# PeterSutor/ADMM-Project

Hardware: AMD Instinct MI355X
Metric: ADMM iterations/sec (lasso 100k x 10k, fp64) (higher is better)
Workload: dtype f64; 1 GPU; lasso.m cached-factor loop, D 100000x10000 fp64, rho=1, lassotest.m recipe seed=1, domaxiters=1, objevals=0, xsolve=inverse; rows=100000, cols=10000, parallelism=rows1

## Files before the change

admm-project_amd/_lib.py:

```python
from __future__ import annotations

import ctypes as C
import os

_HERE = os.path.dirname(os.path.abspath(__file__))
LIB_PATH = os.path.join(_HERE, "libadmm_hip.so")

ABI_VERSION = 5

OK, E_INVALID, E_UNSUPPORTED, E_DEVICE, E_NUMERIC, E_COMM, E_CAPACITY = 0, -1, -2, -3, -4, -5, -6

PROB_LASSO, PROB_LASSO_CONSENSUS, PROB_LAD, PROB_HUBERFIT = 1, 2, 3, 4
PROB_LINEARSVM, PROB_TOTALVARIATION, PROB_QP_BOUNDED, PROB_BASISPURSUIT = 5, 6, 7, 8
PROB_MODEL, PROB_LINEARPROGRAM, PROB_QP_STANDARD, PROB_TV2D = 9, 10, 11, 12
PROB_COVSEL = 13
LOSS_HINGE, LOSS_01, LOSS_HINGE_OBJ01, LOSS_LOGISTIC = 0, 1, 2, 3
LOSS_SQHINGE = 5


def loss_code(text):
    if text in ("hinge", "01"):
        return LOSS_HINGE if text == "hinge" else LOSS_01
    if isinstance(text, str) and text.lower() == "logistic":
        return LOSS_LOGISTIC
# ... 254 lines not shown
 SLM_F_DERR) = range(1, 9)


class LassoMultiDesc(C.Structure):
    _fields_ = [("struct_size", C.c_int32), ("K", C.c_int32), ("m", C.c_int64), ("n", C.c_int64), ("D", _dp),
                ("ldD", C.c_int64), ("S", _dp), ("ns", C.c_int32), ("device", C.c_int32), ("rho", C.c_double),
                ("xsolve", C.c_int32), ("reserved0", C.c_int32), ("lam", _dp), ("ridge", _dp),
                ("nonneg", C.POINTER(C.c_int32)), ("weights", _dp), ("comm", C.c_void_p)]


class LassoMultiOptions(C.Structure):
    _fields_ = [("struct_size", C.c_int32), ("maxiters", C.c_int32), ("rho", C.c_double), ("abstol", C.c_double),
                ("reltol", C.c_double), ("relax", C.c_double), ("fast", C.c_int32), ("convtest", C.c_int32),
                ("domaxiters", C.c_int32), ("objevals", C.c_int32), ("check_every", C.c_int32),
                ("nodualerror", C.c_int32), ("x0", _dp), ("z0", _dp), ("u0", _dp)]


class LassoMultiSummary(C.Structure):
    _fields_ = [("steps", C.c_int32), ("stopped_early", C.c_int32), ("objopt", C.c_double), ("xsolve", C.c_int32),
                ("reserved0", C.c_int32)]


(LM_F_XOPT, LM_F_ZOPT, LM_F_UOPT, LM_F_PNORM, LM_F_PERR, LM_F_OBJEVALS, LM_F_DNORM, LM_F_DERR) = range(1, 9)


class CovselMultiDesc(C.Structure):
    _fields_ = [("struct_size", C.c_int32), ("K", C.c_int32), ("m", C.c_int64), ("n", C.c_int64), ("D", _dp),
                ("ldD", C.c_int64), ("S", _dp), ("lam", _dp), ("device", C.c_int32), ("reserved0", C.c_int32),
                ("comm", C.c_void_p)]


class CovselMultiOptions(C.Structure):
    _fields_ = [("struct_size", C.c_int32), ("maxiters", C.c_int32), ("rho", C.c_double), ("abstol", C.c_double),
                ("reltol", C.c_double), ("relax", C.c_double), ("fast", C.c_int32), ("convtest", C.c_int32),
                ("domaxiters", C.c_int32), ("objevals", C.c_int32), ("check_every", C.c_int32),
                ("nodualerror", C.c_int32), ("rhos", _dp), ("z0", _dp), ("u0", _dp)]


class CovselMultiSummary(C.Structure):
    _fields_ = [("steps", C.c_int32), ("stopped_early", C.c_int32), ("objopt", C.c_double),
                ("jacobi_sweeps", C.c_int32), ("reserved0", C.c_int32)]


(CM_F_XOPT, CM_F_ZOPT, CM_F_UOPT, CM_F_PNORM, CM_F_PERR, CM_F_OBJEVALS, CM_F_DNORM, CM_F_DERR, CM_F_COV) = range(1, 10)
COVSEL_SMALL_MAX = 96


class L1ClassDesc(C.Structure):
    _fields_ = [("struct_size", C.c_int32), ("K", C.c_int32), ("m", C.c_int64), ("n", C.c_int64), ("D", _dp),
                ("ldD", C.c_int64), ("ELL", _dp), ("nell", C.c_int32), ("device", C.c_int32), ("C", C.c_double),
                ("xsolve", C.c_int32), ("reserved0", C.c_int32), ("loss", C.POINTER(C.c_int32)), ("lam", _dp),
                ("ridge", _dp), ("nonneg", C.POINTER(C.c_int32)), ("l1weights", _dp), ("comm", C.c_void_p)]


class L1ClassOptions(C.Structure):
    _fields_ = list(LassoMultiOptions._fields_)


class L1ClassSummary(C.Structure):
    _fields_ = list(LassoMultiSummary._fields_)


(L1C_F_XOPT, L1C_F_ZOPT, L1C_F_UOPT, L1C_F_PNORM, L1C_F_PERR, L1C_F_OBJEVALS, L1C_F_DNORM, L1C_F_DERR) = range(1, 9)


class SparseL1ClassDesc(C.Structure):
    _fields_ = [("struct_size", C.c_int32), ("K", C.c_int32), ("D", C.POINTER(SparseDesc)), ("ELL", _dp),
                ("nell", C.c_int32), ("device", C.c_int32), ("C", C.c_double), ("xsolve", C.c_int32),
                ("reserved0", C.c_int32), ("loss", C.POINTER(C.c_int32)), ("lam", _dp), ("ridge", _dp),
                ("nonneg", C.POINTER(C.c_int32)), ("l1weights", _dp), ("comm", C.c_void_p)]


class SparseL1ClassOptions(C.Structure):
    _fields_ = list(SparseRegOptions._fields_)


class SparseL1ClassSummary(C.Structure):
    _fields_ = [("steps", C.c_int32), ("stopped_early", C.c_int32), ("objopt", C.c_double), ("xsolve", C.c_int32),
                ("reserved0", C.c_int32), ("cg_iters_total", C.c_int64), ("cg_capped_updates", C.c_int64)]


FIELD_NUMERIC, FIELD_TEXT, FIELD_HANDLE, FIELD_SPARSE, FIELD_OTHER = 0, 1, 2, 3, 4
RES_FETCH, RES_SCALAR, RES_START = 0, 1, 2
STORAGE_FP64, STORAGE_COMPACT = 0, 1
F_WVALS = 23
F_COVSEL_S = 24
F_TV2D_ROW_STAGE = 25
F_SPARSE_NNZ = 26
TV2D_ROWS_AUTO, TV2D_ROWS_GREEN, TV2D_ROWS_COOP, TV2D_ROWS_DCT, TV2D_ROWS_THOMAS = range(5)
TV2D_ROWS_NAMES = ("cg", "green", "coop", "dct", "thomas")


class AdmmError(RuntimeError):
    def __init__(self, code, message):
        super().__init__(f"[admm_hip {code}] {message}")
        self.code = code


_SIGNATURES = {
    "admm_abi_version": (C.c_int, []),
    "admm_last_error": (C.c_char_p, []),
    "admm_device_count": (C.c_int, [C.POINTER(C.c_int)]),
    "admm_device_info": (C.c_int, [C.c_int, C.c_char_p, C.c_size_t, C.POINTER(C.c_int64), C.POINTER(C.c_int32)]),
    "admm_options_default": (None, [C.POINTER(Options)]),
    "admm_problem_desc_default": (None, [C.POINTER(ProblemDesc)]),
    "admm_engine_create": (C.c_int, [C.POINTER(ProblemDesc), C.POINTER(C.c_void_p)]),
    "admm_engine_create_sparse": (C.c_int, [C.POINTER(ProblemDesc), C.POINTER(SparseDesc), C.POINTER(C.c_void_p)]),
    "admm_engine_set_callbacks": (C.c_int, [C.c_void_p, PROX_CALLBACK, C.c_void_p, PROX_CALLBACK, C.c_void_p,
                                            OBJ_CALLBACK, C.c_void_p]),
    "admm_engine_set_operators": (C.c_int, [C.c_void_p, OPERATOR_CALLBACK, C.c_void_p, OPERATOR_CALLBACK, C.c_void_p]),
    "admm_engine_set_constraint_b": (C.c_int, [C.c_void_p, C.POINTER(C.c_double), C.c_int64, C.c_int64, C.c_int32,
                                               C.c_double, OPERATOR_CALLBACK, C.c_void_p]),
    "admm_engine_set_groups": (C.c_int, [C.c_void_p, C.POINTER(C.c_int64), C.c_int32, _dp]),
    "admm_engine_set_penalty": (C.c_int, [C.c_void_p, C.POINTER(PenaltyDesc)]),
    "admm_engine_get_penalty": (C.c_int, [C.c_void_p, C.POINTER(PenaltyDesc), C.POINTER(C.c_int32)]),
    "admm_engine_set_loss": (C.c_int, [C.c_void_p, C.POINTER(LossDesc)]),
    "admm_engine_get_loss": (C.c_int, [C.c_void_p, C.POINTER(LossDesc), C.POINTER(C.c_int32)]),
    "admm_engine_set_svm_cost": (C.c_int, [C.c_void_p, C.POINTER(SvmCostDesc)]),
    "admm_engine_get_svm_cost": (C.c_int, [C.c_void_p, C.POINTER(SvmCostDesc), C.POINTER(C.c_int32)]),
    "admm_engine_set_tv2d_isotropic": (C.c_int, [C.c_void_p, C.c_int32]),
    "admm_engine_run": (C.c_int, [C.c_void_p, C.POINTER(Options), C.POINTER(RunSummary)]),
    "admm_engine_fetch": (C.c_int, [C.c_void_p, C.c_int, _dp, C.c_size_t, C.POINTER(C.c_size_t)]),
    "admm_engine_set_hooks": (C.c_int, [C.c_void_p, ALTU_CALLBACK, C.c_void_p, NORMS_CALLBACK, C.c_void_p]),
    "admm_engine_info": (C.c_int, [C.c_void_p, C.POINTER(EngineInfo)]),
    "admm_engine_xsolve_storage": (C.c_int, [C.c_void_p, C.POINTER(C.c_int32), C.POINTER(C.c_int64),
                                             C.POINTER(C.c_double), C.POINTER(C.c_double), C.POINTER(C.c_double)]),
    "admm_xsolve_compact_accept": (C.c_int, [C.c_double, C.c_double, C.c_double]),
    "admm_tv2d_row_stage": (C.c_int, [C.c_int64, C.c_int64, C.c_double]),
    "admm_tv2d_rows_green_taps": (C.c_int, [C.c_double]),
    "admm_dct_tables": (C.c_int, [C.c_int64, _dp, _dp, _dp, _dp, _dp, C.POINTER(C.c_int64)]),
    "admm_engine_setup_seconds": (C.c_int, [C.c_void_p, C.POINTER(C.c_double)]),
    "admm_engine_kernel_time": (C.c_int, [C.c_void_p, C.c_int, C.POINTER(C.c_double), C.POINTER(C.c_int64)]),
    "admm_engine_set_profiling": (C.c_int, [C.c_void_p, C.c_int]),
    "admm_engine_set_profiling_stride": (C.c_int, [C.c_void_p, C.c_int]),
    "admm_engine_destroy": (None, [C.c_void_p]),
    "admm_binding_create": (C.c_int, [C.c_char_p, C.POINTER(Field), C.c_int32, C.POINTER(Field), C.c_int32,
                                      C.POINTER(C.c_void_p)]),
    "admm_binding_destroy": (None, [C.c_void_p]),
    "admm_binding_desc": (C.POINTER(ProblemDesc), [C.c_void_p]),
    "admm_binding_sparse": (C.POINTER(SparseDesc), [C.c_void_p]),
    "admm_binding_get_info": (C.c_int, [C.c_void_p, C.POINTER(BindingInfo)]),
    "admm_binding_apply": (C.c_int, [C.c_void_p, C.c_void_p]),
    "admm_binding_options": (C.c_int, [C.c_void_p, C.POINTER(Field), C.c_int32, C.POINTER(Field), C.c_int32,
                                       C.POINTER(Options)]),
    "admm_binding_results": (C.c_int, [C.c_void_p, C.POINTER(Options), C.POINTER(RunSummary), C.POINTER(ResultField),
                                       C.c_int32, C.POINTER(C.c_int32)]),
    "admm_memcpy_d2h": (C.c_int, [C.c_void_p, C.c_void_p, C.c_size_t, C.c_void_p]),
    "admm_memcpy_h2d": (C.c_int, [C.c_void_p, C.c_void_p, C.c_size_t, C.c_void_p]),
    "admm_op_gemv_n": (C.c_int, [_dp, C.c_int64, C.c_int64, C.c_int64, _dp, _dp]),
    "admm_op_gemv_t": (C.c_int, [_dp, C.c_int64, C.c_int64, C.c_int64, _dp, C.c_int64, C.c_int32, _dp, C.c_int64]),
    "admm_op_spmv": (C.c_int, [C.POINTER(SparseDesc), C.c_int, _dp, _dp]),
    "admm_op_gram": (C.c_int, [_dp, C.c_int64, C.c_int64, C.c_int64, C.c_double, _dp]),
    "admm_op_cholesky": (C.c_int, [_dp, C.c_int64, C.c_int64]),
    "admm_op_trsv_pair": (C.c_int, [_dp, C.c_int64, C.c_int64, _dp, _dp]),
    "admm_op_soft_threshold": (C.c_int, [_dp, C.c_int64, C.c_double, _dp]),
    "admm_op_pair_soft_threshold": (C.c_int, [_dp, C.c_int64, C.c_double, _dp]),
    "admm_op_group_soft_threshold": (C.c_int, [_dp, C.c_int64, C.POINTER(C.c_int64), C.c_int32, _dp, C.c_double, _dp]),
    "admm_op_penalty_prox": (C.c_int, [_dp, C.c_int64, C.POINTER(C.c_int64), C.c_int32, _dp, C.c_double,
                                       C.POINTER(PenaltyDesc), C.c_double, _dp]),
    "admm_op_loss_prox": (C.c_int, [_dp, C.c_int64, C.c_int32, C.POINTER(LossDesc), C.c_double, _dp]),
    "admm_op_svm_prox": (C.c_int, [_dp, _dp, C.c_int64, C.c_int32, C.c_double, C.c_double, C.POINTER(SvmCostDesc), _dp]),
    "admm_op_symv": (C.c_int, [_dp, C.c_int64, C.c_int64, _dp, C.c_int32, C.c_int64, C.c_int32, _dp]),
    "admm_op_symv_compact": (C.c_int, [_dp, C.c_int64, C.c_int64, _dp, C.c_int32, C.c_int64, C.c_int32, _dp, _dp,
                                       C.c_int64]),
    "admm_op_symv_batch": (C.c_int, [_dp, C.c_int64, C.c_int64, C.c_int32, _dp, C.c_int64, C.c_int64, _dp, C.c_int64]),
    "admm_op_gemm": (C.c_int, [C.c_int32, C.c_int32, C.c_int64, C.c_int64, C.c_int64, C.c_double, _dp, C.c_int64, _dp,
                               C.c_int64, C.c_double, _dp, C.c_int64, C.c_int32]),
    "admm_op_trtri": (C.c_int, [_dp, C.c_int64, C.c_int64, _dp, C.c_int64]),
    "admm_op_llt_apply": (C.c_int, [_dp, C.c_int64, C.c_int64, _dp, _dp]),
    "admm_op_dct_cols": (C.c_int, [_dp, C.c_int64, C.c_int64, C.c_int32, _dp]),
    "admm_op_tv2d_rows": (C.c_int, [_dp, C.c_int64, C.c_int64, C.c_double, C.c_int32, _dp]),
    "admm_op_tv2d_xsolve": (C.c_int, [_dp, C.c_int64, C.c_int64, C.c_double, C.c_int32, _dp]),
    "admm_op_consensus_tail": (C.c_int, [C.c_int32, C.c_int64, C.c_int32, C.c_int32, C.c_double, C.c_double, _dp, _dp,
                                         _dp, _dp, _dp, _dp, _dp, C.c_int32, _dp, _dp, _dp, _dp, _dp, _dp]),
    "admm_comm_unique_id": (C.c_int, [C.c_char_p]),
    "admm_comm_init": (C.c_int, [C.c_char_p, C.c_int, C.c_int, C.c_int, C.c_int, C.POINTER(C.c_void_p)]),
    "admm_comm_info": (C.c_int, [C.c_void_p, C.POINTER(C.c_int), C.POINTER(C.c_int), C.POINTER(C.c_int)]),
    "admm_comm_allreduce_sum": (C.c_int, [C.c_void_p, _dp, C.c_size_t]),
    "admm_comm_measure_latency": (C.c_int, [C.c_void_p, C.c_size_t, C.c_int, C.POINTER(C.c_double)]),
    "admm_comm_destroy": (None, [C.c_void_p]),
    "admm_comm_init_all": (C.c_int, [C.c_int, C.POINTER(C.c_int), C.c_int, C.POINTER(C.c_void_p)]),
    "admm_engine_create_all": (C.c_int, [C.c_int, C.POINTER(ProblemDesc), C.POINTER(C.c_void_p)]),
    "admm_engine_run_all": (C.c_int, [C.c_int, C.POINTER(C.c_void_p), C.POINTER(Options), C.c_int,
                                      C.POINTER(RunSummary)]),
    "admm_svm_ovr_desc_default": (None, [C.POINTER(SvmOvrDesc)]),
    "admm_svm_ovr_options_default": (None, [C.POINTER(SvmOvrOptions)]),
    "admm_svm_ovr_create": (C.c_int, [C.POINTER(SvmOvrDesc), C.POINTER(C.c_void_p)]),
    "admm_svm_ovr_run": (C.c_int, [C.c_void_p, C.POINTER(SvmOvrOptions), C.POINTER(SvmOvrSummary),
                                   C.POINTER(C.c_double)]),
    "admm_svm_ovr_fetch": (C.c_int, [C.c_void_p, C.c_int, _dp, C.c_size_t, C.POINTER(C.c_size_t)]),
    "admm_svm_ovr_set_cost": (C.c_int, [C.c_void_p, _dp, _dp]),
    "admm_svm_ovr_chunk": (C.c_int, []),
    "admm_svm_ovr_destroy": (None, [C.c_void_p]),
    "admm_reg_multi_desc_default": (None, [C.POINTER(RegMultiDesc)]),
    "admm_reg_multi_options_default": (None, [C.POINTER(RegMultiOptions)]),
    "admm_reg_multi_create": (C.c_int, [C.POINTER(RegMultiDesc), C.POINTER(C.c_void_p)]),
    "admm_reg_multi_run": (C.c_int, [C.c_void_p, C.POINTER(RegMultiOptions), C.POINTER(RegMultiSummary),
                                     C.POINTER(C.c_double)]),
    "admm_reg_multi_fetch": (C.c_int, [C.c_void_p, C.c_int, _dp, C.c_size_t, C.POINTER(C.c_size_t)]),
    "admm_reg_multi_set_weights": (C.c_int, [C.c_void_p, _dp]),
    "admm_reg_multi_launches": (C.c_int, [C.c_void_p, C.POINTER(C.c_int64)]),
    "admm_reg_multi_chunk": (C.c_int, []),
    "admm_reg_multi_destroy": (None, [C.c_void_p]),
    "admm_op_spmm": (C.c_int, [C.POINTER(SparseDesc), C.c_int, C.c_int, _dp, _dp]),
    "admm_op_spmm_weighted": (C.c_int, [C.POINTER(SparseDesc), C.c_int32, _dp, _dp, C.c_int32, C.POINTER(C.c_int32),
                                        C.POINTER(C.c_int32), _dp]),
    "admm_op_spmm_cg": (C.c_int, [C.POINTER(SparseDesc), C.c_int32, _dp, _dp, C.c_double, C.c_double, C.c_int32,
                                  C.c_int32, C.POINTER(C.c_int32), _dp, _dp, C.POINTER(C.c_int64),
                                  C.POINTER(C.c_int32)]),
    "admm_sparse_svm_desc_default": (None, [C.POINTER(SparseSvmDesc)]),
    "admm_sparse_svm_options_default": (None, [C.POINTER(SparseSvmOptions)]),
    "admm_sparse_svm_create": (C.c_int, [C.POINTER(SparseSvmDesc), C.POINTER(C.c_void_p)]),
    "admm_sparse_svm_run": (C.c_int, [C.c_void_p, C.POINTER(SparseSvmOptions), C.POINTER(SparseSvmSummary),
                                      C.POINTER(C.c_double)]),
    "admm_sparse_svm_fetch": (C.c_int, [C.c_void_p, C.c_int, _dp, C.c_size_t, C.POINTER(C.c_size_t)]),
    "admm_sparse_svm_set_cost": (C.c_int, [C.c_void_p, _dp, _dp]),
    "admm_sparse_svm_chunk": (C.c_int, []),
    "admm_sparse_svm_destroy": (None, [C.c_void_p]),
    "admm_sparse_reg_desc_default": (None, [C.POINTER(SparseRegDesc)]),
    "admm_sparse_reg_options_default": (None, [C.POINTER(SparseRegOptions)]),
    "admm_sparse_reg_create": (C.c_int, [C.POINTER(SparseRegDesc), C.POINTER(C.c_void_p)]),
    "admm_sparse_reg_run": (C.c_int, [C.c_void_p, C.POINTER(SparseRegOptions), C.POINTER(SparseRegSummary),
                                      C.POINTER(C.c_double)]),
    "admm_sparse_reg_fetch": (C.c_int, [C.c_void_p, C.c_int, _dp, C.c_size_t, C.POINTER(C.c_size_t)]),
    "admm_sparse_reg_set_weights": (C.c_int, [C.c_void_p, _dp]),
    "admm_sparse_reg_chunk": (C.c_int, []),
    "admm_sparse_reg_destroy": (None, [C.c_void_p]),
    "admm_sparse_lasso_desc_default": (None, [C.POINTER(SparseLassoDesc)]),
    "admm_sparse_lasso_options_default": (None, [C.POINTER(SparseLassoOptions)]),
    "admm_sparse_lasso_create": (C.c_int, [C.POINTER(SparseLassoDesc), C.POINTER(C.c_void_p)]),
    "admm_sparse_lasso_run": (C.c_int, [C.c_void_p, C.POINTER(SparseLassoOptions), C.POINTER(SparseLassoSummary),
                                        C.POINTER(C.c_double)]),
    "admm_sparse_lasso_fetch": (C.c_int, [C.c_void_p, C.c_int, _dp, C.c_size_t, C.POINTER(C.c_size_t)]),
    "admm_sparse_lasso_set_weights": (C.c_int, [C.c_void_p, _dp]),
    "admm_sparse_lasso_set_groups": (C.c_int, [C.c_void_p, C.c_int32, C.POINTER(C.c_int64), _dp, _dp]),
    "admm_sparse_lasso_set_observations": (C.c_int, [C.c_void_p, _dp, C.c_int32, C.POINTER(C.c_int32),
                                                     C.POINTER(C.c_int32)]),
    "admm_sparse_lasso_heldout": (C.c_int, [C.c_void_p, _dp, _dp]),
    "admm_sparse_lasso_chunk": (C.c_int, []),
    "admm_sparse_lasso_destroy": (None, [C.c_void_p]),
    "admm_lasso_multi_desc_default": (None, [C.POINTER(LassoMultiDesc)]),
    "admm_lasso_multi_options_default": (None, [C.POINTER(LassoMultiOptions)]),
    "admm_lasso_multi_create": (C.c_int, [C.POINTER(LassoMultiDesc), C.POINTER(C.c_void_p)]),
    "admm_lasso_multi_run": (C.c_int, [C.c_void_p, C.POINTER(LassoMultiOptions), C.POINTER(LassoMultiSummary),
                                       C.POINTER(C.c_double)]),
    "admm_lasso_multi_fetch": (C.c_int, [C.c_void_p, C.c_int, _dp, C.c_size_t, C.POINTER(C.c_size_t)]),
    "admm_lasso_multi_set_weights": (C.c_int, [C.c_void_p, _dp]),
# ... 95 lines not shown
```

admm-project_amd/csrc/dev/symv_packed.hip:

```cpp
#include "../symv.hip"

#include <cstdio>
#include <cstdlib>
#include <string>
#include <vector>

using namespace admm;
constexpr int kSyTile = kTile;

#define CK(e)                                                                   \
  do {                                                                          \
    hipError_t _e = (e);                                                        \
    if (_e != hipSuccess) {                                                     \
      fprintf(stderr, "%s:%d %s\n", __FILE__, __LINE__, hipGetErrorString(_e)); \
      exit(1);                                                                  \
    }                                                                           \
  } while (0)

__global__ void fill_sym(double* M, int64_t n, int64_t ld) {
  const int64_t j = blockIdx.x;
  for (int64_t i = threadIdx.x; i < n; i += blockDim.x) {
    const int64_t a = i > j ? i : j, b = i > j ? j : i;
    M[j * ld + i] = 1e-3 * static_cast<double>((a * 131 + b * 7) % 1009 - 504) + (i == j ? 3.0 : 0.0);
  }
// ... 262 lines not shown
  s.n = n - c0;
  s.r = 2 * lane;
  const int64_t gr = w0 + 2 * lane;
  s.xr0 = x[gr < n ? gr : n - 1];
  s.xr1 = x[gr + 1 < n ? gr + 1 : n - 1];
  double* __restrict__ tout = tpart + static_cast<int64_t>(bi) * ldp + c0;
  double n0 = 0.0, n1 = 0.0;
  if (bi == bj) sy_tile<true, true>(s, 0, n0, n1, tout, lane);
  else if (t < ncached) sy_tile<false, false>(s, 0, n0, n1, tout, lane);
  else sy_tile<false, true>(s, 0, n0, n1, tout, lane);
  *reinterpret_cast<double2_t*>(npart + static_cast<int64_t>(bj) * ldp + gr) = double2_t{n0, n1};
}

template <int MODE>
__global__ __launch_bounds__(kWave) void symv_lower_hybrid(const double* __restrict__ M, int64_t n, int64_t ld,
                                                           const double* __restrict__ x, double* __restrict__ npart,
                                                           double* __restrict__ tpart, int64_t ldp, unsigned ncached) {
  if (blockIdx.x < blockIdx.y) return;
  const unsigned lin = blockIdx.x * (blockIdx.x + 1u) / 2u + blockIdx.y;
  const bool cached = MODE == 0 ? lin < ncached : (lin & 15u) < ncached;
  const int lane = threadIdx.x & 63;
  const int64_t w0 = static_cast<int64_t>(blockIdx.x) * kSyTile;
  const int64_t c0 = static_cast<int64_t>(blockIdx.y) * kSyTile;
  SyLane s;
  s.M = M;
  s.x = x;
  s.ld = ld;
  s.n = n;
  s.r = static_cast<int>(w0) + 2 * lane;
  s.xr0 = x[s.r < n ? s.r : n - 1];
  s.xr1 = x[s.r + 1 < n ? s.r + 1 : n - 1];
  double* __restrict__ tout = tpart + static_cast<int64_t>(blockIdx.x) * ldp;
  double n0 = 0.0, n1 = 0.0;
  if (blockIdx.x == blockIdx.y) sy_tile<true, true>(s, c0, n0, n1, tout, lane);
  else if (cached) sy_tile<false, false>(s, c0, n0, n1, tout, lane);
  else sy_tile<false, true>(s, c0, n0, n1, tout, lane);
  *reinterpret_cast<double2_t*>(npart + static_cast<int64_t>(blockIdx.y) * ldp + s.r) = double2_t{n0, n1};
}

int main(int argc, char** argv) {
  const int64_t n = argc > 1 ? atoll(argv[1]) : 10000;
  const SymvPlan p = symv_plan(n);
  const int64_t ld = p.npad;
  const unsigned nt = static_cast<unsigned>(p.ntile), ntri = nt * (nt + 1) / 2;
  double *M, *P, *x, *np_, *tp, *y, *y2;
  CK(hipMalloc(&M, sizeof(double) * ld * p.npad));
  CK(hipMemset(M, 0, sizeof(double) * ld * p.npad));
  CK(hipMalloc(&P, sizeof(double) * ntri * kSyTile * kSyTile));
  CK(hipMalloc(&x, sizeof(double) * p.npad));
  CK(hipMalloc(&np_, sizeof(double) * nt * p.ldp));
  CK(hipMalloc(&tp, sizeof(double) * nt * p.ldp));
  CK(hipMalloc(&y, sizeof(double) * p.npad));
  CK(hipMalloc(&y2, sizeof(double) * p.npad));
  std::vector<double> hx(p.npad, 0.0);
  for (int64_t i = 0; i < n; ++i) hx[i] = 0.25 + 0.001 * (i % 97);
  CK(hipMemcpy(x, hx.data(), sizeof(double) * p.npad, hipMemcpyHostToDevice));
  hipLaunchKernelGGL(fill_sym, dim3(n), dim3(256), 0, 0, M, n, ld);
  hipLaunchKernelGGL(pack_tiles, dim3(ntri), dim3(256), 0, 0, M, ld, P);
  CK(hipDeviceSynchronize());
  printf("n=%lld tiles=%u packed %.1f MB (padded square %.1f MB)\n", (long long)n, ntri, ntri * 131072e-6,
         8e-6 * ld * p.npad);
  hipEvent_t e0, e1;
  CK(hipEventCreate(&e0));
  CK(hipEventCreate(&e1));
  const int reps = 60;
  double last_us = 0.0;
  auto time_it = [&](const char* name, auto&& launch, double* yout) {
    CK(hipMemset(np_, 0, sizeof(double) * nt * p.ldp));
    CK(hipMemset(tp, 0, sizeof(double) * nt * p.ldp));
    for (int i = 0; i < 5; ++i) launch();
    CK(hipEventRecord(e0));
    for (int i = 0; i < reps; ++i) launch();
    CK(hipEventRecord(e1));
    CK(hipEventSynchronize(e1));
    float ms;
    CK(hipEventElapsedTime(&ms, e0, e1));
    hipLaunchKernelGGL(symv_reduce_kernel, dim3(ceil_div(n, 16)), dim3(kBlock), 0, 0, np_, tp, p.ldp, n, p.ntile, yout,
                       nullptr);
    CK(hipDeviceSynchronize());
    const double us = ms * 1e3 / reps;
    last_us = us;
    printf("%-44s %8.2f us  %6.3f TB/s\n", name, us, ntri * 131072.0 / us * 1e-6);
  };
  if (argc > 2 && std::string(argv[2]) == "compact") {
    SymvPlan pf = p, pc = p;
    pf.packed = pc.packed = pc.compact = true;
    double* C;
    CK(hipMalloc(&C, sizeof(double) * symv_compact_elems(pc)));
    launch_symv_compact_pack(pc, P, 0, true, C, nullptr, 0);
    pc.scales = symv_compact_scales(pc, C);
    CK(hipDeviceSynchronize());
    const double cmb = symv_tile_prefix_bytes(pc, ntri) * 1e-6;
    printf("compact storage %.1f MB (TB/s column: fp64 algorithmic bytes over time)\n", cmb);
    std::vector<double> h1(n), h2(n);
    for (int round = 0; round < 2; ++round)
      for (int64_t mb : {0, 64, 105, 136, 168, 200, 232, 264, 290, 320}) {
        char nm[96];
        pf.ncached = symv_cached_tiles(pf, mb << 20);
        pc.ncached = symv_cached_tiles(pc, mb << 20);
        snprintf(nm, sizeof nm, "fp64    %3lld MB cacheable (%lld tiles)", (long long)mb, (long long)pf.ncached);
        time_it(nm, [&] { launch_symv_lower(pf, P, 0, x, np_, tp, y, nullptr, 0, 0, 1, false); }, y);
        snprintf(nm, sizeof nm, "compact %3lld MB cacheable (%lld tiles)", (long long)mb, (long long)pc.ncached);
        time_it(nm, [&] { launch_symv_lower(pc, C, 0, x, np_, tp, y2, nullptr, 0, 0, 1, false); }, y2);
        printf("   compact over stored bytes: %6.3f TB/s\n", cmb / last_us);
      }
    CK(hipMemcpy(h1.data(), y, sizeof(double) * n, hipMemcpyDeviceToHost));
    CK(hipMemcpy(h2.data(), y2, sizeof(double) * n, hipMemcpyDeviceToHost));
    double err = 0, ymax = 0;
    for (int64_t i = 0; i < n; ++i) err = fmax(err, fabs(h1[i] - h2[i])), ymax = fmax(ymax, fabs(h1[i]));
    printf("max |y_compact - y_fp64| / max |y| = %.3e\n", err / ymax);
    return 0;
  }
  time_it("column-major padded (production)", [&] {
    hipLaunchKernelGGL(symv_lower_kernel<false>, dim3(nt, nt), dim3(kWave), 0, 0, M, n, ld, x, np_, tp, p.ldp, 0, 1, 0u,
                       nullptr, nullptr);
  }, y);
  time_it("tile-packed, NT", [&] {
    hipLaunchKernelGGL((symv_packed_kernel<true, 0>), dim3(ntri), dim3(kWave), 0, 0, P, n, x, np_, tp, p.ldp, nt);
  }, y2);
  std::vector<double> h1(n), h2(n);
  CK(hipMemcpy(h1.data(), y, sizeof(double) * n, hipMemcpyDeviceToHost));
  CK(hipMemcpy(h2.data(), y2, sizeof(double) * n, hipMemcpyDeviceToHost));
  double err = 0;
  for (int64_t i = 0; i < n; ++i) err = fmax(err, fabs(h1[i] - h2[i]));
  printf("max |y_packed - y_colmajor| = %.3e\n", err);
  time_it("tile-packed, NT, reversed order", [&] {
    hipLaunchKernelGGL((symv_packed_kernel<true, 1>), dim3(ntri), dim3(kWave), 0, 0, P, n, x, np_, tp, p.ldp, nt);
  }, y2);
  time_it("tile-packed, default loads", [&] {
    hipLaunchKernelGGL((symv_packed_kernel<false, 0>), dim3(ntri), dim3(kWave), 0, 0, P, n, x, np_, tp, p.ldp, nt);
  }, y2);
  for (unsigned nc : {0u, 400u, 800u, 1200u, 1500u, 1800u, 2200u, 3160u}) {
    char nm[96];
    snprintf(nm, sizeof nm, "tile-packed hybrid: %u tiles (%.0f MB) cacheable", nc, nc * 0.131072);
    time_it(nm, [&] {
      hipLaunchKernelGGL(symv_hybrid_kernel, dim3(ntri), dim3(kWave), 0, 0, P, n, x, np_, tp, p.ldp, nc);
    }, y2);
  }
  for (unsigned nc : {0u, 800u, 1200u, 1500u, 1800u}) {
    char nm[96];
    snprintf(nm, sizeof nm, "column-major hybrid: first %u tiles cacheable", nc);
    time_it(nm, [&] {
      hipLaunchKernelGGL(symv_lower_hybrid<0>, dim3(nt, nt), dim3(kWave), 0, 0, M, n, ld, x, np_, tp, p.ldp, nc);
    }, y2);
  }
  for (unsigned nc : {4u, 6u, 7u, 8u, 9u}) {
    char nm[96];
    snprintf(nm, sizeof nm, "column-major hybrid: %u of 16 tiles cacheable", nc);
    time_it(nm, [&] {
      hipLaunchKernelGGL(symv_lower_hybrid<1>, dim3(nt, nt), dim3(kWave), 0, 0, M, n, ld, x, np_, tp, p.ldp, nc);
    }, y2);
  }
  hipLaunchKernelGGL(pack_blocked, dim3(ntri), dim3(256), 0, 0, M, ld, P);
  CK(hipDeviceSynchronize());
#define BLK(DEPTH, OCC)                                                                                               \
  time_it("lane-blocked depth " #DEPTH " occ " #OCC, [&] {                                                            \
    hipLaunchKernelGGL((symv_blocked_kernel<true, DEPTH, OCC>), dim3(ntri), dim3(kWave), 0, 0, P, n, x, np_, tp,      \
                       p.ldp);                                                                                        \
  }, y2);                                                                                                             \
  CK(hipMemcpy(h2.data(), y2, sizeof(double) * n, hipMemcpyDeviceToHost));                                            \
  err = 0;                                                                                                            \
  for (int64_t i = 0; i < n; ++i) err = fmax(err, fabs(h1[i] - h2[i]));                                               \
  printf("   max |y - y_colmajor| = %.3e\n", err);
  BLK(8, 1)
  BLK(16, 1)
  BLK(32, 1)
  BLK(8, 2)
  BLK(16, 2)
  BLK(16, 3)
  BLK(8, 4)
#define PERS(DEPTH, W)                                                                                               \
  {                                                                                                                   \
    char nm[96];                                                                                                      \
    snprintf(nm, sizeof nm, "persistent depth %d waves %u", DEPTH, static_cast<unsigned>(W));                        \
    time_it(nm, [&] {                                                                                                 \
      hipLaunchKernelGGL((symv_persist_kernel<true, DEPTH>), dim3(W), dim3(kWave), 0, 0, P, n, x, np_, tp, p.ldp,    \
                         ntri);                                                                                       \
    }, y2);                                                                                                           \
    CK(hipMemcpy(h2.data(), y2, sizeof(double) * n, hipMemcpyDeviceToHost));                                          \
    err = 0;                                                                                                          \
    for (int64_t i = 0; i < n; ++i) err = fmax(err, fabs(h1[i] - h2[i]));                                             \
    printf("   max |y - y_colmajor| = %.3e\n", err);                                                                 \
  }
  PERS(8, ntri)
  PERS(8, (ntri + 1) / 2)
  PERS(16, (ntri + 1) / 2)
  PERS(8, (ntri + 2) / 3)
  PERS(16, (ntri + 2) / 3)
  PERS(16, (ntri + 3) / 4)
  PERS(8, 2048)
  PERS(16, 1024)
  {
    SymvPlan pp = p;
// ... 21 lines not shown
```

admm-project_amd/csrc/engine.hip:

```cpp
#include "engine_internal.h"
#include "loop_kernels.h"

namespace admm {

static thread_local std::string g_last_error;
void set_error(const std::string& msg) { g_last_error = msg; }
int fail(int code, const std::string& msg) {
  g_last_error = msg;
  return code;
}

EnvSwitches env_switches() {
  EnvSwitches s{};
  s.graph = std::getenv("ADMM_HIP_GRAPH") != nullptr;
  const char* form = std::getenv("ADMM_TRSV_FORM");
  s.trsv_form = !form ? -1 : form[0] == 'b' ? kTrsvBlocked : form[0] == 'o' ? kTrsvOne : -1;
  const char* split = std::getenv("ADMM_HIP_XSPLIT");
  s.xsplit = !split ? -1 : split[0] == '1' ? 1 : 0;
  s.no_unwrapped_fused = std::getenv("ADMM_HIP_NO_UNWRAPPED_FUSED") != nullptr;
  s.no_onepass = std::getenv("ADMM_HIP_NO_ONEPASS") != nullptr;
  return s;
}

int upload(DevMem& mem, double** dst, const double* src, size_t elems, int memkind, hipStream_t stream) {
// ... 221 lines not shown
        [&](const double* y, double* x) { launch_trsv_pair(f.trsv, y, x, nullptr, e->stream); }, &e1, &eb, &diff);
  if (rc != ADMM_OK) {
    e->mem.free_one(work1);
    return rc;
  }
  f.err_trsv_one = e1;
  if (!f.probed) f.err_trsv = eb;
  const bool ok = forced_one || (e1 <= std::max(1e-11, 4.0 * eb) && diff <= std::max(1e-11, 8.0 * eb));
  if (ok) {
    e->mem.free_one(f.work);
    f.work = work1;
    f.trsv = one;
  } else {
    e->mem.free_one(work1);
  }
  return ADMM_OK;
}

int build_slice_factor(admm_engine* e, SliceFactor& f, double* W, int64_t n, int64_t ld, int want, const double* Lgiven,
                       int memkind) {
  f.F = W;
  f.n = n;
  f.ld = ld;
  const int64_t nblk = ceil_div(n, 64);
  ADMM_TRY(e->mem.alloc(&f.dinv, static_cast<size_t>(nblk) * 64 * 64));
  if (Lgiven) {
    ADMM_HIP_TRY(hipMemsetAsync(W, 0, sizeof(double) * ld * n, e->stream));
    ADMM_HIP_TRY(hipMemcpy2DAsync(W, ld * sizeof(double), Lgiven, n * sizeof(double), n * sizeof(double), n,
                                  memkind == ADMM_MEM_DEVICE ? hipMemcpyDeviceToDevice : hipMemcpyHostToDevice,
                                  e->stream));
    launch_trtri_diag(W, n, ld, f.dinv, e->stream);
  } else {
    double* infod = nullptr;
    ADMM_TRY(e->mem.alloc(&infod, 1));
    int32_t* info_dev = reinterpret_cast<int32_t*>(infod);
    ADMM_TRY(cholesky_lower(W, n, ld, info_dev, f.dinv, e->stream));
    int32_t info = 0;
    ADMM_HIP_TRY(hipMemcpyAsync(&info, info_dev, sizeof(int32_t), hipMemcpyDeviceToHost, e->stream));
    ADMM_HIP_TRY(hipStreamSynchronize(e->stream));
    e->mem.free_one(infod);
    if (info != 0) {
      f.chol_info = info;
      return fail(ADMM_E_NUMERIC, "Cholesky failed: matrix must be positive definite (pivot " + std::to_string(info) + ")");
    }
  }
  {
    std::vector<double> dg(static_cast<size_t>(n));
    ADMM_HIP_TRY(hipMemcpy2DAsync(dg.data(), sizeof(double), W, (ld + 1) * sizeof(double), sizeof(double), n,
                                  hipMemcpyDeviceToHost, e->stream));
    ADMM_HIP_TRY(hipStreamSynchronize(e->stream));
    double lo = INFINITY, hi = 0.0;
    for (double v : dg) {
      lo = v < lo ? v : lo;
      hi = v > hi ? v : hi;
    }
    f.diag_min = lo;
    f.diag_max = hi;
    f.cond_diag = (lo > 0.0) ? (hi / lo) * (hi / lo) : INFINITY;
  }
  if (want == ADMM_XSOLVE_AUTO) want = ADMM_XSOLVE_INVERSE;
  ADMM_TRY(e->mem.alloc(&f.work, trsv_plan_elems(n)));
  ADMM_TRY(trsv_build(W, n, ld, f.dinv, f.work, &f.trsv, e->stream));
  f.mode = ADMM_XSOLVE_TRSV;
  if (want == ADMM_XSOLVE_INVERSE) {
    ADMM_TRY(build_explicit_inverse(e, f));
    ADMM_TRY(probe_and_choose(e, f));
    if (f.mode == ADMM_XSOLVE_INVERSE) {
      e->mem.free_one(f.work);
      f.work = nullptr;
      f.trsv = TrsvPlan{};
    } else {
      e->mem.free_one(f.Minv);
      f.Minv = nullptr;
    }
  }
  if (f.mode == ADMM_XSOLVE_TRSV) ADMM_TRY(choose_trsv_form(e, f));
  return ADMM_OK;
}

bool symv_compact_accept(double err_compact, double err_fp64, double diff) {
  return err_compact <= std::max(1e-11, 4.0 * err_fp64) && diff <= std::max(1e-11, 8.0 * err_fp64);
}

static int choose_symv_storage(admm_engine* e, SliceFactor& f) {
  if (f.mode != ADMM_XSOLVE_INVERSE || !f.Minv || !f.F || f.pinv || !f.planSy.packed || f.planSy.compact ||
      f.n < kSymvHalfMin || e->sy_split || e->keep_fp64)
    return ADMM_OK;
  if (!stream_hint(symv_tile_prefix_bytes(f.planSy, symv_tiles(f.planSy)))) return ADMM_OK;
  SymvPlan cp = f.planSy;
  cp.compact = true;
  double* C = nullptr;
  ADMM_TRY(e->mem.alloc(&C, symv_compact_elems(cp)));
  launch_symv_compact_pack(cp, f.Minv, 0, true, C, nullptr, e->stream);
  cp.scales = symv_compact_scales(cp, C);
  cp.ncached = symv_cached_tiles(cp, kSymvCacheBytes);
  double ea = NAN, eb = NAN, diff = NAN;
  const int rc = probe_two_forms(
      e, f, [&](const double* y, double* x) { launch_symv_lower(cp, C, 0, y, e->syN, e->syT, x, nullptr, e->stream); },
      [&](const double* y, double* x) { apply_inverse(e, f, y, x, nullptr); }, &ea, &eb, &diff);
  if (rc != ADMM_OK) {
    e->mem.free_one(C);
    return rc;
  }
  f.err_cq = ea;
  f.err_cq_ref = eb;
  f.cq_diff = diff;
  if (symv_compact_accept(ea, eb, diff)) {
    e->mem.free_one(f.Minv);
    f.Minv = C;
    f.planSy = cp;
  } else {
    e->mem.free_one(C);
  }
  return ADMM_OK;
}

void release_slice_factor(admm_engine* e, SliceFactor& f) {
  e->mem.free_one(f.Minv);
  e->mem.free_one(f.work);
  e->mem.free_one(f.dinv);
  f = SliceFactor{};
}

void apply_slice_factor(admm_engine* e, const SliceFactor& f, const double* y, double* out) {
  if (f.mode == ADMM_XSOLVE_INVERSE) apply_inverse(e, f, y, out, e->ctrl);
  else launch_trsv_pair(f.trsv, y, out, e->ctrl, e->stream);
}

static int decide_sy_split(admm_engine* e) {
  const SliceFactor& f = e->xfac;
  e->sy_split = false;
  const int nr = e->comm ? comm_nranks(e->comm) : 1;
  if (nr <= 1 || f.mode != ADMM_XSOLVE_INVERSE || f.n < kSymvHalfMin) return ADMM_OK;
  double* probe = e->syN;
  for (int k = 0; k < 3; ++k) ADMM_TRY(comm_allreduce_device(e->comm, probe, static_cast<size_t>(f.n), e->stream));
  ADMM_HIP_TRY(hipStreamSynchronize(e->stream));
  const auto c0 = std::chrono::steady_clock::now();
  const int reps = 10;
  for (int k = 0; k < reps; ++k) ADMM_TRY(comm_allreduce_device(e->comm, probe, static_cast<size_t>(f.n), e->stream));
  ADMM_HIP_TRY(hipStreamSynchronize(e->stream));
  double lat_us = std::chrono::duration<double>(std::chrono::steady_clock::now() - c0).count() * 1e6 / reps;
  ADMM_TRY(allreduce_scalar(e, &lat_us, probe));
  lat_us /= nr;
  const double t_us = 4.0 * static_cast<double>(f.planSy.npad) * static_cast<double>(f.planSy.npad) / 6.4e6;
  e->sy_split = t_us * (1.0 - 1.0 / nr) > 1.15 * lat_us + 8.0;
  if (const int forced = env_switches().xsplit; forced >= 0) e->sy_split = forced == 1;
  ADMM_HIP_TRY(hipMemsetAsync(e->syN, 0, sizeof(double) * f.planSy.npart_elems(), e->stream));
  ADMM_HIP_TRY(hipMemsetAsync(e->syT, 0, sizeof(double) * f.planSy.tpart_elems(), e->stream));
  return ADMM_OK;
}

int build_unwrapped_pinv(admm_engine* e, const double* Dp_given) {
  const int64_t m = e->m, n = e->n;
  if (env_switches().no_unwrapped_fused) return ADMM_OK;
  if (!uw_supported(m, n) || (e->comm && comm_nranks(e->comm) > 1)) return ADMM_OK;
  if (static_cast<double>(m) * static_cast<double>(n) * 8.0 > 1.5e9) return ADMM_OK;
  const int64_t ldp = round_up(n, 2);
  if (Dp_given) {
    ADMM_TRY(e->mem.alloc(&e->Dp, static_cast<size_t>(ldp) * m));
    ADMM_HIP_TRY(hipMemcpy2DAsync(e->Dp, ldp * sizeof(double), Dp_given, n * sizeof(double), n * sizeof(double), m,
                                  hipMemcpyDeviceToDevice, e->stream));
  } else {
    SliceFactor& f = e->xfac;
    if (e->xsolve_requested == ADMM_XSOLVE_TRSV || e->xsolve_requested == ADMM_XSOLVE_CG) return ADMM_OK;
    SliceFactor tmp{};
    const double* Minv = nullptr;
    int64_t ldM = 0;
    if (f.mode == ADMM_XSOLVE_INVERSE && f.Minv && !f.planSy.packed) {
      Minv = f.Minv;
      ldM = f.ldM;
    } else if (f.mode == ADMM_XSOLVE_TRSV && !f.probed && f.F) {
      tmp.F = f.F;
      tmp.n = f.n;
      tmp.ld = f.ld;
      tmp.dinv = f.dinv;
      ADMM_TRY(build_explicit_inverse(e, tmp, false));
      Minv = tmp.Minv;
      ldM = tmp.ldM;
    } else {
      return ADMM_OK;
    }
    ADMM_TRY(e->mem.alloc(&e->Dp, static_cast<size_t>(ldp) * m));
    ADMM_HIP_TRY(hipMemsetAsync(e->Dp, 0, sizeof(double) * ldp * m, e->stream));
    launch_gemm(0, 1, n, m, n, 1.0, Minv, ldM, e->D, e->ldD, 0.0, e->Dp, ldp, false, e->stream);
    ADMM_HIP_TRY(hipStreamSynchronize(e->stream));
    if (tmp.Minv) e->mem.free_one(tmp.Minv);
  }
  e->ldDp = ldp;
  e->uwR = uw_rows_per_block(m);
  e->uwnblk = static_cast<int32_t>(ceil_div(m, static_cast<int64_t>(e->uwR)));
// ... 417 lines not shown
  if (!src) return fail(ADMM_E_INVALID, "field not available for this run");
  if (cap < count) return fail(ADMM_E_CAPACITY, "destination too small");
  if (count) ADMM_HIP_TRY(hipMemcpy(dst, src, count * sizeof(double), hipMemcpyDeviceToHost));
  if (written) *written = count;
  return ADMM_OK;
}

int admm_memcpy_d2h(void* host_dst, const void* device_src, size_t bytes, void* hip_stream) {
  if ((!host_dst || !device_src) && bytes) return fail(ADMM_E_INVALID, "NULL argument");
  hipStream_t st = static_cast<hipStream_t>(hip_stream);
  ADMM_HIP_TRY(hipMemcpyAsync(host_dst, device_src, bytes, hipMemcpyDeviceToHost, st));
  ADMM_HIP_TRY(hipStreamSynchronize(st));
  return ADMM_OK;
}

int admm_memcpy_h2d(void* device_dst, const void* host_src, size_t bytes, void* hip_stream) {
  if ((!device_dst || !host_src) && bytes) return fail(ADMM_E_INVALID, "NULL argument");
  hipStream_t st = static_cast<hipStream_t>(hip_stream);
  ADMM_HIP_TRY(hipMemcpyAsync(device_dst, host_src, bytes, hipMemcpyHostToDevice, st));
  ADMM_HIP_TRY(hipStreamSynchronize(st));
  return ADMM_OK;
}

int admm_engine_info(admm_engine* e, admm_engine_info_t* info) {
  if (!e || !info) return fail(ADMM_E_INVALID, "NULL argument");
  if (info->struct_size != static_cast<int32_t>(sizeof(admm_engine_info_t)))
    return fail(ADMM_E_INVALID, "admm_engine_info_t.struct_size mismatch (ABI version skew)");
  const SliceFactor* f = &e->xfac;
  if (e->problem == ADMM_PROB_LASSO_CONSENSUS && !e->cslices.empty()) f = &e->cslices[0].fac;
  const bool has = f->F != nullptr || f->Minv != nullptr;
  info->xsolve_requested = e->xsolve_requested;
  info->xsolve_used = has ? f->mode : e->xsolve;
  info->pinv_used = f->pinv ? 1 : 0;
  info->probed = f->probed ? 1 : 0;
  info->factor_n = has ? f->n : 0;
  info->rank = f->pinv ? f->rank : (has ? f->n : 0);
  info->trsv_blocks = (has && f->mode == ADMM_XSOLVE_TRSV) ? f->trsv.nblk : 0;
  info->jacobi_sweeps = (e->problem == ADMM_PROB_COVSEL) ? static_cast<int32_t>(e->cov_sweeps) : f->jacobi_sweeps;
  info->unwrapped_fused = e->Dp ? 1 : 0;
  info->cond_estimate = has ? f->cond_diag : NAN;
  info->probe_err_inverse = f->probed ? f->err_inv : NAN;
  info->probe_err_trsv = (f->probed || f->err_trsv_one == f->err_trsv_one) ? f->err_trsv : NAN;
  info->probe_err_trsv_one = f->err_trsv_one;
  info->probe_diff = f->probed ? f->probe_diff : NAN;
  auto tally = [&](const SliceFactor& s) {
    const int64_t tile_bytes = int64_t{8} * 128 * 128;
    if (s.mode == ADMM_XSOLVE_INVERSE && s.Minv && s.n >= kSymvHalfMin) {
      const int64_t tiles = symv_tiles(s.planSy);
      const int64_t cached = std::min<int64_t>(tiles, std::max<int64_t>(0, s.planSy.ncached));
      const int64_t cbytes = symv_tile_prefix_bytes(s.planSy, cached);
      info->xsolve_cacheable_bytes += cbytes;
      info->xsolve_stream_bytes += symv_tile_prefix_bytes(s.planSy, tiles) - cbytes;
    } else if (s.mode == ADMM_XSOLVE_INVERSE && s.Minv) {
      info->xsolve_cacheable_bytes += int64_t{8} * s.n * s.n;
    } else if (s.mode == ADMM_XSOLVE_TRSV && s.trsv.one) {
      const int64_t nt = s.trsv.ntile, tiles = nt * (nt + 1) / 2;
      const int64_t cached = s.trsv.streaming ? std::min<int64_t>(tiles, std::max<int64_t>(0, s.trsv.ncached)) : tiles;
      info->xsolve_cacheable_bytes += 2 * cached * tile_bytes;
      info->xsolve_stream_bytes += 2 * (tiles - cached) * tile_bytes;
    } else if (s.mode == ADMM_XSOLVE_TRSV && s.trsv.Fm) {
      const int64_t nt = s.trsv.ntile, tiles = nt * (nt + 1) / 2;
      const int64_t cached = s.trsv.streaming ? std::min<int64_t>(tiles, std::max<int64_t>(0, s.trsv.ncached)) : tiles;
      info->xsolve_cacheable_bytes += 2 * cached * tile_bytes;
      info->xsolve_stream_bytes += 2 * (tiles - cached) * tile_bytes;
    }
  };
  info->obj_bound_max = e->obj_bound_seen;
  info->obj_form_literal = (e->obj_alt && e->obj_auto && e->obj_gram_bad) ? 1 : 0;
  info->ngroups = e->ngroups;
  info->xsolve_cacheable_bytes = info->xsolve_stream_bytes = 0;
  if (e->problem == ADMM_PROB_LASSO_CONSENSUS) {
    for (const ConsSlice& sl : e->cslices) tally(sl.fac);
  } else if (has) {
    tally(*f);
  }
  return ADMM_OK;
}

int admm_engine_xsolve_storage(admm_engine* e, int32_t* form, int64_t* stored_bytes, double* probe_err_compact,
                               double* probe_err_fp64, double* probe_diff) {
  if (!e) return fail(ADMM_E_INVALID, "engine is NULL");
  const SliceFactor& f = e->xfac;
  const bool inv = f.mode == ADMM_XSOLVE_INVERSE && f.Minv;
  if (form) *form = (inv && f.planSy.compact) ? ADMM_STORAGE_COMPACT : ADMM_STORAGE_FP64;
  if (stored_bytes) {
    *stored_bytes = 0;
    if (inv && f.planSy.packed) *stored_bytes = symv_tile_prefix_bytes(f.planSy, symv_tiles(f.planSy));
    else if (inv) *stored_bytes = int64_t{8} * f.ldM * f.planSy.npad;
  }
  if (probe_err_compact) *probe_err_compact = f.err_cq;
  if (probe_err_fp64) *probe_err_fp64 = f.err_cq_ref;
  if (probe_diff) *probe_diff = f.cq_diff;
  return ADMM_OK;
}

int admm_xsolve_compact_accept(double err_compact, double err_fp64, double diff) {
  return symv_compact_accept(err_compact, err_fp64, diff) ? 1 : 0;
}

int admm_engine_setup_seconds(admm_engine* e, double* seconds) {
  if (!e || !seconds) return fail(ADMM_E_INVALID, "NULL argument");
  *seconds = e->setup_seconds;
  return ADMM_OK;
}

int admm_engine_set_profiling(admm_engine* e, int enabled) {
  if (!e) return fail(ADMM_E_INVALID, "engine is NULL");
  e->profiling = enabled < 0 ? 0xffffffffu : static_cast<uint32_t>(enabled);
  return ADMM_OK;
}

int admm_engine_set_profiling_stride(admm_engine* e, int stride) {
  if (!e || stride < 1) return fail(ADMM_E_INVALID, "bad argument");
  e->prof_stride = stride;
  return ADMM_OK;
}

int admm_engine_kernel_time(admm_engine* e, int which, double* total_ms, int64_t* launches) {
  if (!e || which < 0 || which >= ADMM_K_COUNT) return fail(ADMM_E_INVALID, "bad argument");
  if (total_ms) *total_ms = e->timers[which].total_ms;
  if (launches) *launches = e->timers[which].launches;
  return ADMM_OK;
}

void admm_engine_destroy(admm_engine* e) {
  if (!e) return;
  (void)hipSetDevice(e->device);
  if (e->stream) (void)hipStreamSynchronize(e->stream);
  free_hist(e);
  for (auto& t : e->timers)
    for (hipEvent_t ev : t.ev) (void)hipEventDestroy(ev);
  e->mem.release();
  sparse_device_free(&e->sp);
  if (e->ctrl_host) (void)hipHostFree(e->ctrl_host);
  if (e->cg_st_host) (void)hipHostFree(e->cg_st_host);
  if (e->stream) (void)hipStreamDestroy(e->stream);
  delete e;
}

}
```

admm-project_amd/csrc/kernels.h:

```cpp
#pragma once
#include <vector>

#include "common.h"

namespace admm {

struct GemvNPlan {
  int64_t m, n, ld;
  int64_t ldy;
  int32_t nchunk;
  int64_t cols_per_chunk;
  size_t part_elems() const { return static_cast<size_t>(nchunk) * ldy; }
};
GemvNPlan gemv_n_plan(int64_t m, int64_t n, int64_t ld);
void launch_gemv_n(const GemvNPlan& p, const double* D, const double* x, double* ypart, const Ctrl* ctrl,
                   hipStream_t stream);
void launch_sum_partials(const double* part, int32_t nchunk, int64_t ld, int64_t len, double* y, const Ctrl* ctrl,
                         hipStream_t stream);

struct GemvTPlan {
  int64_t m, n, ld;
  int64_t ldg;
  int32_t nchunk;
  int32_t rows_per_chunk;
  size_t part_elems(int nrhs) const { return static_cast<size_t>(nchunk) * nrhs * ldg; }
};
GemvTPlan gemv_t_plan(int64_t m, int64_t n, int64_t ld);
void launch_gemv_t(const GemvTPlan& p, const double* D, const double* v0, const double* v1, const double* v2,
                   int nrhs, double* gpart, const Ctrl* ctrl, hipStream_t stream);
void launch_sum_partials_t(const GemvTPlan& p, const double* gpart, int nrhs, double* g, int64_t ldg_out,
                           const Ctrl* ctrl, hipStream_t stream);

struct SymvPlan {
  int64_t n, npad;
  int64_t ldp;
  int32_t ntile;
  bool packed;
  int64_t ncached;
  bool compact;
  const double* scales;
  size_t npart_elems() const { return static_cast<size_t>(ntile) * ldp; }
  size_t tpart_elems() const { return static_cast<size_t>(ntile) * ldp; }
};
SymvPlan symv_plan(int64_t n);
constexpr int64_t kSymvCacheBytes = int64_t{168} << 20;
int64_t symv_tiles(const SymvPlan& p);
size_t symv_packed_elems(const SymvPlan& p);
int64_t symv_cached_tiles(const SymvPlan& p, int64_t budget_bytes);
struct FinArgs;
void launch_symv_lower_batch(const SymvPlan& p, const double* const* Ms_dev, int32_t K, const double* x0, int64_t xstride,
                             double* npart0, double* tpart0, int64_t pstride, const Ctrl* ctrl, hipStream_t stream,
                             const FinArgs* fin = nullptr);
void launch_symv_pack(const SymvPlan& p, const double* M, int64_t ld, double* P, hipStream_t stream);
int64_t symv_tile_prefix_bytes(const SymvPlan& p, int64_t t);
size_t symv_compact_elems(const SymvPlan& p);
double* symv_compact_scales(const SymvPlan& p, double* C);
void launch_symv_compact_pack(const SymvPlan& p, const double* M, int64_t ld, bool src_packed, double* C, double* deq,
                              hipStream_t stream);
void launch_symv_small(const double* M, int64_t n, int64_t ld, const double* x, double* y, const Ctrl* ctrl,
                       hipStream_t stream);
void launch_symv_lower(const SymvPlan& p, const double* M, int64_t ld, const double* x, double* npart, double* tpart,
                       double* y, const Ctrl* ctrl, hipStream_t stream, int part_rank = 0, int part_count = 1,
                       bool reduce = true);

struct MultiRec;
size_t symm_part_elems(const SymvPlan& p, int32_t K);
void launch_symm_packed(const SymvPlan& p, const double* P, const double* Y, double* X, double* part,
                        const MultiRec* rec, int32_t K, hipStream_t stream);

void launch_gemm(int transA, int transB, int64_t M, int64_t N, int64_t K, double alpha, const double* A, int64_t lda,
                 const double* B, int64_t ldb, double beta, double* C, int64_t ldc, bool lower_only,
                 hipStream_t stream);
int cholesky_lower(double* A, int64_t n, int64_t lda, int32_t* info_dev, double* dinv, hipStream_t stream);
void launch_trtri_diag(const double* L, int64_t n, int64_t ldl, double* dinv, hipStream_t stream);
int trtri_lower_from_diag(const double* L, int64_t n, int64_t ldl, const double* dinv, double* X, int64_t ldx,
                          hipStream_t stream, bool clear = true);
void launch_llt_apply(const double* L, int64_t n, int64_t ld, const double* x, double* tmp, double* y,
                      hipStream_t stream);
void launch_symmetrize_lower(double* A, int64_t n, int64_t lda, hipStream_t stream);
void launch_add_diag(double* A, int64_t n, int64_t lda, double shift, hipStream_t stream);
void launch_fill(double* p, size_t n, double v, hipStream_t stream);

struct TrsvPlan {
  int64_t n, npad;
  int64_t ldm, ldp;
  int32_t ntile, nblk, bt;
  double* Fm;
  double* Um;
  int64_t ncached;
  double* P[2];
  double *v, *w;
  bool streaming;
  bool one;
  double* X1;
  double *np1, *tp1;
  double* w1;
};
struct Tri1Args {
  const double* X;
  int64_t n;
  const double* y;
  double* npart;
  double* tpart;
  double* w;
  int64_t ldp;
  uint32_t ncached;
  uint32_t ntri;
  int32_t ntile;
};
void launch_tri1_forward(const Tri1Args& a, const FinArgs* fin, bool fin_pending, const Ctrl* ctrl, hipStream_t stream);
void launch_tri1_backward(const Tri1Args& a, const Ctrl* ctrl, hipStream_t stream);
void launch_tri1_reduce(const Tri1Args& a, double* x, const Ctrl* ctrl, hipStream_t stream);
void launch_symv_reduce(const SymvPlan& p, const double* npart, const double* tpart, double* y, const Ctrl* ctrl,
                        hipStream_t stream);
Tri1Args tri1_args(const TrsvPlan& p, const double* y);
void launch_tri1_pair(const TrsvPlan& p, const double* y, double* x, const FinArgs* fin, bool fin_pending,
                      const Ctrl* ctrl, hipStream_t stream);
constexpr int kTrsvBlocked = 0, kTrsvOne = 1;
int trsv_resolve_form(int64_t n, int form);
size_t trsv_plan_elems(int64_t n, int form = kTrsvBlocked);
int trsv_build(const double* L, int64_t n, int64_t ldl, const double* dinv64, double* buf, TrsvPlan* plan,
               hipStream_t stream, int form = kTrsvBlocked);
// ... 13 lines not shown
```

admm-project_amd/csrc/l1class.hip:

```cpp
#include <algorithm>
#include <cmath>
#include <cstddef>
#include <cstring>
#include <string>
#include <vector>

#include "l1class_device.h"
#include "l1class_group_device.h"
#include "multi_host.h"
#include "spmm.h"
#include "svm_cost_device.h"
#include "svm_ovr.h"

namespace admm {

namespace {

constexpr int KC = kSpmmChunk;
static_assert(kSpmmChunk == kOvrChunk, "one chunk for the n x n product and for the passes over D");

constexpr int kFwRows = 64, kFwWaves = 8, kFwThreads = kFwWaves * kWave;
constexpr int kFwPanel = 512;
constexpr int kFwStep = 8;
constexpr int kFwSlots = (KC + kFwWaves - 1) / kFwWaves;
// ... 331 lines not shown
}

}

struct admm_l1class : admm::MultiHost {
  admm_engine* eng = nullptr;
  int64_t m = 0, n = 0, ldz = 0, ldx = 0, ldt = 0;
  int32_t chunks = 0, Kp = 0, nwg_m = 0, nwg_n = 0, tiles_per = 0, nranges = 0, ell_shared = 0;
  double C = 1.0;
  admm::SymvPlan plan{};
  const double* P = nullptr;
  double* spart = nullptr;
  double *ycol = nullptr, *xcol = nullptr;
  double *X = nullptr, *Y = nullptr, *Z2 = nullptr, *U2 = nullptr;
  double *Z1 = nullptr, *U1 = nullptr, *T1 = nullptr, *DZ1 = nullptr, *ELL = nullptr;
  double *gpart = nullptr, *GS = nullptr;
  double *mpart = nullptr, *npart = nullptr;
  double *W = nullptr, *CC = nullptr, *LW = nullptr, *par = nullptr;
  int32_t *loss = nullptr, *nonneg = nullptr;
  std::vector<int32_t> loss_host;
  std::vector<double> cost_host;
  std::vector<char> chunk_logistic;
  double *pnorm = nullptr, *perr = nullptr, *dnorm = nullptr, *derr = nullptr, *objv = nullptr;
  int64_t launches = 0, d_passes = 0;
  admm::GroupMulti grp;
  admm_l1class_options last{};
};

namespace {

using namespace admm;

const char* kPerFit = ": run admm() with A = [D; I] per fit instead";

int l1c_setup(admm_l1class* o, const admm_l1class_desc* desc, const std::vector<double>& ph,
              const std::vector<int32_t>& nh) {
  const int64_t m = desc->m, n = desc->n;
  const int32_t K = desc->K;
  const int64_t me = std::max(m, n);
  std::vector<double> pad, zeros(static_cast<size_t>(me), 0.0);
  admm_problem_desc d;
  admm_problem_desc_default(&d);
  d.problem = ADMM_PROB_LASSO;
  d.m = me;
  d.n = n;
  d.D = desc->D;
  d.ldD = desc->ldD;
  if (me != m) {
    pad.assign(static_cast<size_t>(me) * n, 0.0);
    for (int64_t j = 0; j < n; ++j)
      std::memcpy(pad.data() + j * me, desc->D + j * desc->ldD, sizeof(double) * m);
    d.D = pad.data();
    d.ldD = me;
  }
  d.s = zeros.data();
  d.lambda = 0.0;
  d.rho = 1.0;
  d.xsolve = desc->xsolve;
  d.mem = ADMM_MEM_HOST;
  d.device = desc->device;
  ADMM_TRY(engine_create_keep_fp64(&d, &o->eng));
  admm_engine* e = o->eng;
  o->stream = e->stream;
  o->device = e->device;
  o->K = K;
  o->m = m;
  o->n = n;
  o->C = desc->C;
  o->chunks = spmm_chunks(K);
  o->Kp = o->chunks * KC;
  o->ldz = round_up(m, 2);
  o->ldx = round_up(n, 2);
  o->ldt = round_up(n, 2);
  o->nwg_m = ovr_pass_workgroups(m);
  o->nwg_n = grid_blocks(n, kBlock, kMultiMaxWg);
  {
    const int64_t tiles = ceil_div(m, int64_t{kTrTile}), strips = ceil_div(n, int64_t{kTrTile});
    const int64_t want = std::min<int64_t>(std::max<int64_t>(ceil_div(int64_t{kTrTarget}, strips), 1), tiles);
    o->tiles_per = static_cast<int32_t>(ceil_div(tiles, want));
    o->nranges = static_cast<int32_t>(ceil_div(tiles, int64_t{o->tiles_per}));
  }
  const SliceFactor& f = e->xfac;
  const size_t kp = static_cast<size_t>(o->Kp);
  if (f.mode == ADMM_XSOLVE_INVERSE && f.Minv && !f.pinv && !f.planSy.compact) {
    o->plan = f.planSy;
    if (f.planSy.packed) {
      o->P = f.Minv;
    } else {
      double* P = nullptr;
      ADMM_TRY(o->mem.alloc(&P, symv_packed_elems(o->plan)));
      launch_symv_pack(o->plan, f.Minv, f.ldM, P, o->stream);
      o->plan.packed = true;
      o->P = P;
    }
    ADMM_TRY(o->mem.alloc(&o->spart, symm_part_elems(o->plan, K)));
  } else if (f.mode == ADMM_XSOLVE_TRSV && f.F) {
    for (double** p : {&o->ycol, &o->xcol}) {
      ADMM_TRY(o->mem.alloc(p, static_cast<size_t>(o->ldt) * K));
      ADMM_HIP_TRY(hipMemsetAsync(*p, 0, sizeof(double) * o->ldt * K, o->stream));
    }
  } else {
    return fail(ADMM_E_UNSUPPORTED, std::string("the engine built no n x n form of the x-update for this D") + kPerFit);
  }
  for (double** p : {&o->X, &o->Y, &o->Z2, &o->U2}) {
    ADMM_TRY(o->mem.alloc(p, kp * n));
    ADMM_HIP_TRY(hipMemsetAsync(*p, 0, sizeof(double) * kp * n, o->stream));
  }
  for (double** p : {&o->Z1, &o->U1, &o->T1, &o->DZ1}) {
    ADMM_TRY(o->mem.alloc(p, kp * o->ldz));
    ADMM_HIP_TRY(hipMemsetAsync(*p, 0, sizeof(double) * kp * o->ldz, o->stream));
  }
  o->ell_shared = desc->nell == 1 && K > 1 ? 1 : 0;
  const int32_t ecols = o->ell_shared ? 1 : K;
  ADMM_TRY(o->mem.alloc(&o->ELL, static_cast<size_t>(ecols) * o->ldz));
  ADMM_HIP_TRY(hipMemsetAsync(o->ELL, 0, sizeof(double) * ecols * o->ldz, o->stream));
  ADMM_TRY(upload_cols(*o, o->ELL, o->ldz, desc->ELL, m, ecols, ADMM_MEM_HOST));
  ADMM_TRY(o->mem.alloc(&o->gpart, static_cast<size_t>(o->nranges) * 3 * kp * o->ldx));
  ADMM_TRY(o->mem.alloc(&o->GS, 3 * kp * o->ldx));
  ADMM_HIP_TRY(hipMemsetAsync(o->GS, 0, sizeof(double) * 3 * kp * o->ldx, o->stream));
  ADMM_TRY(o->mem.alloc(&o->mpart, kp * LM_COUNT * kMultiMaxWg));
  ADMM_HIP_TRY(hipMemsetAsync(o->mpart, 0, sizeof(double) * kp * LM_COUNT * kMultiMaxWg, o->stream));
  ADMM_TRY(o->mem.alloc(&o->npart, kp * LN_COUNT * kMultiMaxWg));
  ADMM_HIP_TRY(hipMemsetAsync(o->npart, 0, sizeof(double) * kp * LN_COUNT * kMultiMaxWg, o->stream));
  ADMM_TRY(o->mem.alloc(&o->par, static_cast<size_t>(2) * K));
  ADMM_HIP_TRY(hipMemcpyAsync(o->par, ph.data(), sizeof(double) * 2 * K, hipMemcpyHostToDevice, o->stream));
  ADMM_TRY(alloc_words(*o, &o->nonneg, static_cast<size_t>(K)));
  ADMM_HIP_TRY(hipMemcpyAsync(o->nonneg, nh.data(), sizeof(int32_t) * K, hipMemcpyHostToDevice, o->stream));
  o->loss_host.assign(static_cast<size_t>(K), ADMM_LOSS_LOGISTIC);
  if (desc->loss) o->loss_host.assign(desc->loss, desc->loss + K);
  o->chunk_logistic.assign(static_cast<size_t>(o->chunks), 0);
  for (int32_t k = 0; k < K; ++k)
    if (o->loss_host[k] == ADMM_LOSS_LOGISTIC) o->chunk_logistic[k / KC] = 1;
  ADMM_TRY(alloc_words(*o, &o->loss, static_cast<size_t>(K)));
  ADMM_HIP_TRY(hipMemcpyAsync(o->loss, o->loss_host.data(), sizeof(int32_t) * K, hipMemcpyHostToDevice, o->stream));
  o->cost_host.assign(static_cast<size_t>(2 * K), 1.0);
  ADMM_TRY(o->mem.alloc(&o->CC, static_cast<size_t>(2 * K)));
  ADMM_HIP_TRY(hipMemcpyAsync(o->CC, o->cost_host.data(), sizeof(double) * 2 * K, hipMemcpyHostToDevice, o->stream));
  ADMM_TRY(alloc_common(*o));
  ADMM_HIP_TRY(hipStreamSynchronize(o->stream));
  ADMM_HIP_TRY(hipGetLastError());
  if (desc->l1weights) ADMM_TRY(set_shared_weights(*o, n, desc->l1weights, &o->LW));
  return ADMM_OK;
}

int l1c_upload_stacked(admm_l1class* o, const double* src, double* V1, double* V2) {
  const size_t kp = static_cast<size_t>(o->Kp);
  if (!src) {
    ADMM_HIP_TRY(hipMemsetAsync(V1, 0, sizeof(double) * kp * o->ldz, o->stream));
    ADMM_HIP_TRY(hipMemsetAsync(V2, 0, sizeof(double) * kp * o->n, o->stream));
    return ADMM_OK;
  }
  const int64_t mn = o->m + o->n;
  ADMM_HIP_TRY(hipMemcpy2DAsync(V1, o->ldz * sizeof(double), src, mn * sizeof(double), o->m * sizeof(double), o->K,
                                hipMemcpyHostToDevice, o->stream));
  std::vector<double> hb(kp * o->n);
  spmm_pack(src + o->m, mn, o->n, o->K, hb.data());
  ADMM_HIP_TRY(hipMemcpyAsync(V2, hb.data(), sizeof(double) * hb.size(), hipMemcpyHostToDevice, o->stream));
  ADMM_HIP_TRY(hipStreamSynchronize(o->stream));
  return ADMM_OK;
}

int l1c_fetch_n(admm_l1class* o, const double* src, double* dst, int64_t ld) {
  std::vector<double> hb(static_cast<size_t>(o->Kp) * o->n);
  ADMM_HIP_TRY(hipMemcpy(hb.data(), src, sizeof(double) * hb.size(), hipMemcpyDeviceToHost));
  spmm_unpack(hb.data(), o->n, o->K, dst, ld);
  return ADMM_OK;
}
// ... 328 lines not shown
```

admm-project_amd/csrc/lasso_multi.hip:

```cpp
#include <algorithm>
#include <cmath>
#include <cstddef>
#include <cstring>
#include <string>
#include <vector>

#include "group_multi.h"
#include "multi_host.h"
#include "sparse_lasso.h"

namespace admm {

namespace {

constexpr int KC = kSpmmChunk;

__global__ __launch_bounds__(kBlock) void lm_gather_kernel(const double* __restrict__ V, int64_t n, int32_t K,
                                                           double* __restrict__ col, int64_t ld) {
  const int64_t i = static_cast<int64_t>(blockIdx.x) * kBlock + threadIdx.x;
  const int32_t k = blockIdx.y;
  if (i < n) col[k * ld + i] = V[(static_cast<int64_t>(k / KC) * n + i) * KC + k % KC];
}

__global__ __launch_bounds__(kBlock) void lm_scatter_kernel(const double* __restrict__ col, int64_t ld, int64_t n,
// ... 10 lines not shown

struct admm_lasso_multi : MultiHost {
  admm_engine* eng = nullptr;
  int64_t m = 0, n = 0, ldt = 0;
  int32_t ns = 1, chunks = 0, nwg_n = 0, nwg_m = 0;
  double rho = 1.0;
  SymvPlan plan{};
  const double* P = nullptr;
  double* spart = nullptr;
  double *ycol = nullptr, *xcol = nullptr;
  double *X = nullptr, *Y = nullptr, *Z = nullptr, *U = nullptr;
  double* T = nullptr;
  double* S = nullptr;
  double* DTS = nullptr;
  double *part = nullptr, *fpart = nullptr;
  double *W = nullptr, *par = nullptr;
  int32_t* nonneg = nullptr;
  GroupMulti grp;
  double *pnorm = nullptr, *perr = nullptr, *dnorm = nullptr, *derr = nullptr, *objv = nullptr;
  admm_lasso_multi_options last{};
};

namespace {

using namespace admm;

const char* kPerFit = ": run one ADMM_PROB_LASSO engine (admm_engine_create) per fit instead";

int lm_upload(admm_lasso_multi* o, double* dst, const double* src, int64_t rows, int32_t cols, int32_t chunks) {
  const size_t elems = static_cast<size_t>(chunks) * KC * rows;
  if (!src) {
    ADMM_HIP_TRY(hipMemsetAsync(dst, 0, sizeof(double) * elems, o->stream));
    return ADMM_OK;
  }
  std::vector<double> hb(elems);
  spmm_pack(src, rows, rows, cols, hb.data());
  ADMM_HIP_TRY(hipMemcpyAsync(dst, hb.data(), sizeof(double) * elems, hipMemcpyHostToDevice, o->stream));
  ADMM_HIP_TRY(hipStreamSynchronize(o->stream));
  return ADMM_OK;
}

int lm_fetch(admm_lasso_multi* o, const double* src, int64_t rows, double* dst, size_t cap, size_t* written) {
  const size_t need = static_cast<size_t>(rows) * o->K;
  if (cap < need) return fail(ADMM_E_CAPACITY, "destination buffer too small");
  std::vector<double> hb(static_cast<size_t>(o->chunks) * KC * rows);
  ADMM_HIP_TRY(hipMemcpy(hb.data(), src, sizeof(double) * hb.size(), hipMemcpyDeviceToHost));
  spmm_unpack(hb.data(), rows, o->K, dst, rows);
  if (written) *written = need;
  return ADMM_OK;
}

int lm_setup(admm_lasso_multi* o, const admm_lasso_multi_desc* desc, const std::vector<double>& ph,
             const std::vector<int32_t>& nh) {
  const int64_t m = desc->m, n = desc->n;
  const int32_t K = desc->K;
  admm_problem_desc d;
  admm_problem_desc_default(&d);
  d.problem = ADMM_PROB_LASSO;
  d.m = m;
  d.n = n;
  d.D = desc->D;
  d.ldD = desc->ldD;
  d.s = desc->S;
  d.lambda = 0.0;
  d.rho = desc->rho;
  d.xsolve = desc->xsolve;
  d.mem = ADMM_MEM_HOST;
  d.device = desc->device;
  ADMM_TRY(engine_create_keep_fp64(&d, &o->eng));
  admm_engine* e = o->eng;
  o->stream = e->stream;
  o->device = e->device;
  o->K = K;
  o->m = m;
  o->n = n;
  o->ns = desc->ns;
  o->rho = desc->rho;
  o->chunks = spmm_chunks(K);
  o->nwg_n = scg_vec_workgroups(n);
  o->nwg_m = scg_vec_workgroups(m);
  o->ldt = round_up(n, 2);
  const SliceFactor& f = e->xfac;
  const size_t kp = static_cast<size_t>(o->chunks) * KC;
  if (f.mode == ADMM_XSOLVE_INVERSE && f.Minv && !f.pinv && !f.planSy.compact) {
    o->plan = f.planSy;
    if (f.planSy.packed) {
      o->P = f.Minv;
    } else {
      double* P = nullptr;
      ADMM_TRY(o->mem.alloc(&P, symv_packed_elems(o->plan)));
      launch_symv_pack(o->plan, f.Minv, f.ldM, P, o->stream);
      o->plan.packed = true;
      o->P = P;
    }
    ADMM_TRY(o->mem.alloc(&o->spart, symm_part_elems(o->plan, K)));
  } else if (f.mode == ADMM_XSOLVE_TRSV && f.F) {
    for (double** p : {&o->ycol, &o->xcol}) {
      ADMM_TRY(o->mem.alloc(p, static_cast<size_t>(o->ldt) * K));
      ADMM_HIP_TRY(hipMemsetAsync(*p, 0, sizeof(double) * o->ldt * K, o->stream));
    }
  } else {
    return fail(ADMM_E_UNSUPPORTED, std::string("the engine built no n x n form of the x-update for this D") + kPerFit);
  }
  for (double** p : {&o->X, &o->Y, &o->Z, &o->U}) {
    ADMM_TRY(o->mem.alloc(p, kp * n));
    ADMM_HIP_TRY(hipMemsetAsync(*p, 0, sizeof(double) * kp * n, o->stream));
  }
  ADMM_TRY(o->mem.alloc(&o->T, kp * m));
  ADMM_HIP_TRY(hipMemsetAsync(o->T, 0, sizeof(double) * kp * m, o->stream));
  {
    const int32_t sch = o->ns == 1 ? 1 : o->chunks;
    const size_t sp = static_cast<size_t>(sch) * KC;
    ADMM_TRY(o->mem.alloc(&o->S, sp * m));
    ADMM_TRY(o->mem.alloc(&o->DTS, sp * n));
    ADMM_TRY(lm_upload(o, o->S, desc->S, m, o->ns, sch));
    double *sc = nullptr, *gc = nullptr;
    ADMM_TRY(o->mem.alloc(&sc, static_cast<size_t>(m) * o->ns));
    ADMM_TRY(o->mem.alloc(&gc, static_cast<size_t>(n) * o->ns));
    ADMM_HIP_TRY(hipMemcpyAsync(sc, desc->S, sizeof(double) * m * o->ns, hipMemcpyHostToDevice, o->stream));
    launch_gemm(1, 0, n, o->ns, m, 1.0, e->D, e->ldD, sc, m, 0.0, gc, n, false, o->stream);
    std::vector<double> gh(static_cast<size_t>(n) * o->ns);
    ADMM_HIP_TRY(hipMemcpyAsync(gh.data(), gc, sizeof(double) * gh.size(), hipMemcpyDeviceToHost, o->stream));
    ADMM_HIP_TRY(hipStreamSynchronize(o->stream));
    ADMM_TRY(lm_upload(o, o->DTS, gh.data(), n, o->ns, sch));
    o->mem.free_one(sc);
    o->mem.free_one(gc);
  }
  ADMM_TRY(o->mem.alloc(&o->part, kp * SL_COUNT * kScgMaxWg));
  ADMM_HIP_TRY(hipMemsetAsync(o->part, 0, sizeof(double) * kp * SL_COUNT * kScgMaxWg, o->stream));
  ADMM_TRY(o->mem.alloc(&o->fpart, kp * kScgMaxWg));
  ADMM_HIP_TRY(hipMemsetAsync(o->fpart, 0, sizeof(double) * kp * kScgMaxWg, o->stream));
  ADMM_TRY(o->mem.alloc(&o->par, static_cast<size_t>(2) * K));
  ADMM_HIP_TRY(hipMemcpyAsync(o->par, ph.data(), sizeof(double) * 2 * K, hipMemcpyHostToDevice, o->stream));
  ADMM_TRY(alloc_words(*o, &o->nonneg, static_cast<size_t>(K)));
  ADMM_HIP_TRY(hipMemcpyAsync(o->nonneg, nh.data(), sizeof(int32_t) * K, hipMemcpyHostToDevice, o->stream));
  ADMM_TRY(alloc_common(*o));
  ADMM_HIP_TRY(hipStreamSynchronize(o->stream));
  ADMM_HIP_TRY(hipGetLastError());
  if (desc->weights) ADMM_TRY(set_shared_weights(*o, n, desc->weights, &o->W));
  return ADMM_OK;
}

void lm_xupdate(admm_lasso_multi* o) {
  if (o->P) {
    launch_symm_packed(o->plan, o->P, o->Y, o->X, o->spart, o->rec, o->K, o->stream);
    return;
  }
  const dim3 grid(static_cast<unsigned>(ceil_div(o->n, kBlock)), static_cast<unsigned>(o->K));
  hipLaunchKernelGGL(lm_gather_kernel, grid, dim3(kBlock), 0, o->stream, o->Y, o->n, o->K, o->ycol, o->ldt);
  for (int32_t k = 0; k < o->K; ++k)
    launch_trsv_pair(o->eng->xfac.trsv, o->ycol + static_cast<int64_t>(k) * o->ldt,
                     o->xcol + static_cast<int64_t>(k) * o->ldt, nullptr, o->stream);
  hipLaunchKernelGGL(lm_scatter_kernel, grid, dim3(kBlock), 0, o->stream, o->xcol, o->ldt, o->n, o->K, o->rec, o->X);
}

}

extern "C" {

void admm_lasso_multi_desc_default(admm_lasso_multi_desc* d) {
  if (!d) return;
  std::memset(d, 0, sizeof(*d));
  d->struct_size = sizeof(admm_lasso_multi_desc);
  d->K = 1;
  d->ns = 1;
  d->rho = 1.0;
  d->xsolve = ADMM_XSOLVE_AUTO;
// ... 208 lines not shown
```

admm-project_amd/csrc/ops.hip:

```cpp
#include <cstring>
#include <string>
#include <vector>

#include "dct.h"
#include "engine_internal.h"
#include "group_multi.h"
#include "kernels.h"
#include "loop_kernels.h"
#include "multi_device.h"
#include "spmm.h"
#include "tv2d.h"

using namespace admm;

namespace {

struct Scratch {
  std::vector<void*> ptrs;
  ~Scratch() {
    for (void* p : ptrs) (void)hipFree(p);
  }
  template <typename T = double>
  int alloc(T** out, size_t elems) {
    void* p = nullptr;
// ... 411 lines not shown
  }
  return ADMM_OK;
}

int admm_op_symm_packed(const double* M, int64_t n, int64_t ldM, double* X, int32_t K, const int32_t* stop_mask,
                        const double* Y) {
  if (!M || !X || !Y || n <= 0 || ldM < n || K < 1)
    return fail(ADMM_E_INVALID, "symm_packed: bad argument (n >= 1, ldM >= n, K >= 1)");
  ADMM_TRY(need_device());
  Scratch sc;
  SymvPlan plan = symv_plan(n);
  double *dM, *dP, *dX, *dY, *part;
  ADMM_TRY(sc.alloc(&dM, static_cast<size_t>(plan.npad) * plan.npad));
  ADMM_HIP_TRY(hipMemset(dM, 0, sizeof(double) * plan.npad * plan.npad));
  ADMM_TRY(put_padded(dM, plan.npad, M, n, ldM));
  ADMM_TRY(sc.alloc(&dP, symv_packed_elems(plan)));
  launch_symv_pack(plan, dM, plan.npad, dP, nullptr);
  plan.packed = true;
  const size_t elems = static_cast<size_t>(spmm_chunks(K)) * kSpmmChunk * n;
  std::vector<double> hb(elems);
  spmm_pack(Y, n, n, K, hb.data());
  ADMM_TRY(sc.put(&dY, static_cast<const double*>(hb.data()), elems));
  spmm_pack(X, n, n, K, hb.data());
  ADMM_TRY(sc.put(&dX, static_cast<const double*>(hb.data()), elems));
  ADMM_TRY(sc.alloc(&part, symm_part_elems(plan, K)));
  ADMM_HIP_TRY(hipMemset(part, 0xFF, sizeof(double) * symm_part_elems(plan, K)));
  MultiRec* rec = nullptr;
  if (stop_mask) {
    std::vector<MultiRec> rh(static_cast<size_t>(K), MultiRec{0, 0, 0, 0});
    for (int32_t k = 0; k < K; ++k) rh[k].stop = stop_mask[k] != 0;
    ADMM_TRY(sc.put(&rec, static_cast<const MultiRec*>(rh.data()), rh.size()));
  }
  launch_symm_packed(plan, dP, dY, dX, part, rec, K, nullptr);
  ADMM_TRY(fetch(hb.data(), dX, elems));
  spmm_unpack(hb.data(), n, K, X, n);
  return ADMM_OK;
}

int admm_op_group_soft_threshold_multi(const double* V, int64_t n, int32_t K, const int64_t* sizes, int32_t ngroups,
                                       const double* groupweights, const double* t, const int32_t* stop_mask, double* Z) {
  if (!V || !Z || !t || n <= 0 || K < 1)
    return fail(ADMM_E_INVALID, "group_soft_threshold_multi: bad argument (n >= 1, K >= 1)");
  for (int32_t k = 0; k < K; ++k)
    if (!finite_nonneg(t[k]))
      return fail(ADMM_E_INVALID, "group_soft_threshold_multi: t[" + std::to_string(k) + "] is negative or not finite");
  GroupPlanHost h;
  ADMM_TRY(group_plan_build(sizes, ngroups, groupweights, n, kGmLimits, &h));
  ADMM_TRY(need_device());
  Scratch sc;
  const size_t elems = static_cast<size_t>(spmm_chunks(K)) * kSpmmChunk * n;
  std::vector<double> hb(elems);
  double *dV, *dZ, *dplan, *dt;
  spmm_pack(V, n, n, K, hb.data());
  ADMM_TRY(sc.put(&dV, static_cast<const double*>(hb.data()), elems));
  spmm_pack(Z, n, n, K, hb.data());
  ADMM_TRY(sc.put(&dZ, static_cast<const double*>(hb.data()), elems));
  ADMM_TRY(sc.put<double>(&dplan, h.blob.data(), h.blob.size()));
  ADMM_TRY(sc.put(&dt, t, static_cast<size_t>(K)));
  MultiRec* rec = nullptr;
  std::vector<MultiRec> rh(static_cast<size_t>(K), MultiRec{0, 0, 0, 0});
  for (int32_t k = 0; stop_mask && k < K; ++k) rh[k].stop = stop_mask[k] != 0;
  ADMM_TRY(sc.put(&rec, static_cast<const MultiRec*>(rh.data()), rh.size()));
  launch_group_multi_shrink(dV, dZ, K, h.bind(dplan), dt, rec, nullptr);
  ADMM_TRY(fetch(hb.data(), dZ, elems));
  spmm_unpack(hb.data(), n, K, Z, n);
  return ADMM_OK;
}

int admm_group_multi_plan(int64_t n, const int64_t* sizes, int32_t ngroups, int64_t* wg_first, int32_t cap, int32_t* nwg,
                          int64_t* budget) {
  GroupPlanHost h;
  ADMM_TRY(group_plan_build(sizes, ngroups, nullptr, n, kGmLimits, &h));
  if (nwg) *nwg = h.nwg;
  if (budget) *budget = h.budget;
  if (wg_first) {
    if (cap < h.nwg + 1) return fail(ADMM_E_CAPACITY, "destination buffer too small");
    std::memcpy(wg_first, h.blob.data() + h.o_wge, sizeof(int64_t) * (static_cast<size_t>(h.nwg) + 1));
  }
  return ADMM_OK;
}

int admm_op_symv_compact(const double* M, int64_t n, int64_t ldM, const double* x, int32_t fin, int64_t ncached,
                         int32_t part_count, double* y, double* Q, int64_t ldQ) {
  if (!M || !x || !y || n <= 0 || ldM < n || ncached < -1 || part_count < 1 || (Q && ldQ < n))
    return fail(ADMM_E_INVALID, "symv_compact: bad argument (ncached >= -1, part_count >= 1, ldQ >= n)");
  ADMM_TRY(need_device());
  Scratch sc;
  double *dM, *dx, *dy, *dC, *dQ = nullptr, *npart, *tpart;
  ADMM_TRY(sc.alloc(&dx, round_up(n, 2)));
  ADMM_TRY(sc.alloc(&dy, round_up(n, 2)));
  ADMM_HIP_TRY(hipMemcpy(dx, x, sizeof(double) * n, hipMemcpyHostToDevice));
  SymvPlan plan = symv_plan(n);
  plan.packed = plan.compact = true;
  ADMM_TRY(sc.alloc(&dM, static_cast<size_t>(plan.npad) * plan.npad));
  ADMM_HIP_TRY(hipMemset(dM, 0, sizeof(double) * plan.npad * plan.npad));
  ADMM_TRY(put_padded(dM, plan.npad, M, n, ldM));
  ADMM_TRY(sc.alloc(&dC, symv_compact_elems(plan)));
  if (Q) ADMM_TRY(sc.alloc(&dQ, symv_packed_elems(plan)));
  launch_symv_compact_pack(plan, dM, plan.npad, false, dC, dQ, nullptr);
  plan.scales = symv_compact_scales(plan, dC);
  plan.ncached = ncached >= 0 ? ncached : symv_cached_tiles(plan, kSymvCacheBytes);
  ADMM_TRY(sc.alloc(&npart, plan.npart_elems()));
  ADMM_TRY(sc.alloc(&tpart, plan.tpart_elems()));
  Ctrl* ctrl = nullptr;
  if (fin) {
    ADMM_TRY(sc.alloc(&ctrl, 1));
    ADMM_HIP_TRY(hipMemset(ctrl, 0, sizeof(Ctrl)));
  }
  const int fill = part_count > 1 ? 0 : 0xFF;
  std::vector<double> part(static_cast<size_t>(n));
  for (int32_t r = 0; r < part_count; ++r) {
    ADMM_HIP_TRY(hipMemset(npart, fill, sizeof(double) * plan.npart_elems()));
    ADMM_HIP_TRY(hipMemset(tpart, fill, sizeof(double) * plan.tpart_elems()));
    if (fin) launch_symv_lower_fin(plan, dC, dx, npart, tpart, FinArgs{}, false, ctrl, nullptr, r, part_count, dy);
    else launch_symv_lower(plan, dC, 0, dx, npart, tpart, dy, ctrl, nullptr, r, part_count);
    ADMM_HIP_TRY(hipDeviceSynchronize());
    ADMM_HIP_TRY(hipMemcpy(r == 0 ? y : part.data(), dy, sizeof(double) * n, hipMemcpyDeviceToHost));
    if (r > 0)
      for (int64_t i = 0; i < n; ++i) y[i] += part[i];
  }
  if (Q) {
    std::vector<double> P(symv_packed_elems(plan));
    ADMM_HIP_TRY(hipMemcpy(P.data(), dQ, sizeof(double) * P.size(), hipMemcpyDeviceToHost));
    for (int64_t j = 0; j < n; ++j)
      for (int64_t i = j; i < n; ++i) {
        const int64_t bi = i / 128, bj = j / 128, t = bi * (bi + 1) / 2 + bj;
        const double v = P[static_cast<size_t>(t) * 128 * 128 + (j % 128) * 128 + (i % 128)];
        Q[i + j * ldQ] = v;
        Q[j + i * ldQ] = v;
      }
  }
  return ADMM_OK;
}

int admm_op_symv_batch(const double* Ms, int64_t n, int64_t ldM, int32_t K, const double* X, int64_t ldX,
                       int64_t ncached, double* Y, int64_t ldY) {
  if (!Ms || !X || !Y || n <= 0 || ldM < n || K < 1 || ldX < n || ldY < n || ncached < -1)
    return fail(ADMM_E_INVALID, "symv_batch: bad argument (K >= 1, ncached >= -1)");
  ADMM_TRY(need_device());
  Scratch sc;
  SymvPlan plan = symv_plan(n);
  if (ncached >= 0) plan.ncached = ncached;
  plan.packed = true;
  const int64_t npad = plan.npad;
  const size_t pelems = symv_packed_elems(plan), pstride = plan.npart_elems();
  double *dM, *dP, *dX, *dY, *npart, *tpart;
  const double** dptr;
  ADMM_TRY(sc.alloc(&dM, static_cast<size_t>(npad) * npad));
  ADMM_TRY(sc.alloc(&dP, pelems * K));
  ADMM_TRY(sc.alloc(&dptr, K));
  ADMM_TRY(sc.alloc(&dX, static_cast<size_t>(npad) * K));
  ADMM_TRY(sc.alloc(&dY, static_cast<size_t>(npad) * K));
  ADMM_TRY(sc.alloc(&npart, pstride * K));
  ADMM_TRY(sc.alloc(&tpart, pstride * K));
  ADMM_HIP_TRY(hipMemset(dM, 0, sizeof(double) * npad * npad));
  ADMM_HIP_TRY(hipMemset(dX, 0, sizeof(double) * npad * K));
  ADMM_HIP_TRY(hipMemset(npart, 0xFF, sizeof(double) * pstride * K));
  ADMM_HIP_TRY(hipMemset(tpart, 0xFF, sizeof(double) * pstride * K));
  std::vector<const double*> ptrs(static_cast<size_t>(K));
  for (int32_t k = 0; k < K; ++k) {
    ADMM_TRY(put_padded(dM, npad, Ms + static_cast<size_t>(k) * ldM * n, n, ldM));
    launch_symv_pack(plan, dM, npad, dP + pelems * k, nullptr);
    ADMM_HIP_TRY(hipDeviceSynchronize());
    ptrs[k] = dP + pelems * k;
  }
  ADMM_HIP_TRY(hipMemcpy(dptr, ptrs.data(), sizeof(const double*) * K, hipMemcpyHostToDevice));
  ADMM_HIP_TRY(hipMemcpy2D(dX, npad * sizeof(double), X, ldX * sizeof(double), n * sizeof(double), K,
                           hipMemcpyHostToDevice));
  launch_symv_lower_batch(plan, dptr, K, dX, npad, npart, tpart,
                          static_cast<int64_t>(pstride), nullptr, nullptr, nullptr);
  for (int32_t k = 0; k < K; ++k)
    launch_symv_reduce(plan, npart + pstride * k, tpart + pstride * k, dY + npad * k, nullptr, nullptr);
  ADMM_HIP_TRY(hipDeviceSynchronize());
  ADMM_HIP_TRY(hipMemcpy2D(Y, ldY * sizeof(double), dY, npad * sizeof(double), n * sizeof(double), K,
                           hipMemcpyDeviceToHost));
  return ADMM_OK;
// ... 311 lines not shown
```

admm-project_amd/csrc/symv.hip:

```cpp

#include <algorithm>

#include "finalize_device.h"
#include "kernels.h"
#include "slot_reduce.h"
#include "tri_tile.h"

namespace admm {

template <bool PACKED, bool COMPACT = false, int NBUF = 2>
__device__ __forceinline__ void symv_lower_body(unsigned block_x, unsigned block_y, const double* __restrict__ M,
                                                int64_t n, int64_t ld, const double* __restrict__ x,
                                                double* __restrict__ npart, double* __restrict__ tpart, int64_t ldp,
                                                int32_t part_rank, int32_t part_count, uint32_t ncached,
                                                const double* __restrict__ scales = nullptr) {
  static_assert(PACKED || !COMPACT, "the compact storage is tile-packed");
  unsigned bi, bj, lin;
  if (PACKED) {
    lin = block_x;
    tri_decode(lin, bi, bj);
  } else {
    bi = block_x;
    bj = block_y;
    if (bi < bj) return;
    lin = bi * (bi + 1u) / 2u + bj;
  }
  if (part_count > 1 && static_cast<int32_t>(lin % static_cast<unsigned>(part_count)) != part_rank) return;
  const int lane = threadIdx.x & 63;
  const int64_t w0 = static_cast<int64_t>(bi) * kTile;
  const int64_t c0 = static_cast<int64_t>(bj) * kTile;
  const int64_t gr = w0 + 2 * lane;
  SyLane s;
  int64_t cbase;
  double* __restrict__ tout = tpart + static_cast<int64_t>(bi) * ldp;
  if (PACKED) {
    s.M = COMPACT ? reinterpret_cast<const double*>(reinterpret_cast<const char*>(M) + cq_tile_offset(lin, bi))
                  : M + static_cast<int64_t>(lin) * (kTile * kTile);
    s.x = x + c0;
    s.ld = kTile;
    s.n = n - c0;
    s.r = 2 * lane;
    cbase = 0;
    tout += c0;
  } else {
    s.M = M;
    s.x = x;
    s.ld = ld;
    s.n = n;
    s.r = static_cast<int>(gr);
    cbase = c0;
  }
  s.xr0 = x[gr < n ? gr : n - 1];
  s.xr1 = x[gr + 1 < n ? gr + 1 : n - 1];
  double n0 = 0.0, n1 = 0.0;
  if (lin < ncached) {
    if (bi == bj) sy_tile<true, false, true, true, NBUF>(s, cbase, n0, n1, tout, lane);
    else if (COMPACT) sy_tile_cq<false, NBUF>(s, scales[lin], n0, n1, tout, lane);
    else sy_tile<false, false, true, true, NBUF>(s, cbase, n0, n1, tout, lane);
  } else {
    if (bi == bj) sy_tile<true, true, true, true, NBUF>(s, cbase, n0, n1, tout, lane);
    else if (COMPACT) sy_tile_cq<true, NBUF>(s, scales[lin], n0, n1, tout, lane);
    else sy_tile<false, true, true, true, NBUF>(s, cbase, n0, n1, tout, lane);
  }
  *reinterpret_cast<double2_t*>(npart + static_cast<int64_t>(bj) * ldp + gr) = double2_t{n0, n1};
}

template <bool PACKED, bool COMPACT = false>
__global__ __launch_bounds__(kWave) void symv_lower_kernel(const double* __restrict__ M, int64_t n, int64_t ld,
                                                           const double* __restrict__ x, double* __restrict__ npart,
                                                           double* __restrict__ tpart, int64_t ldp,
                                                           int32_t part_rank, int32_t part_count, uint32_t ncached,
                                                           const Ctrl* __restrict__ ctrl,
                                                           const double* __restrict__ scales) {
  if (ctrl && ctrl->stop) return;
  symv_lower_body<PACKED, COMPACT>(blockIdx.x, blockIdx.y, M, n, ld, x, npart, tpart, ldp, part_rank, part_count,
                                   ncached, scales);
}

template <bool COMPACT>
__global__ __launch_bounds__(kWave) void symv_lower_fin_kernel(const double* __restrict__ M, int64_t n,
                                                               const double* __restrict__ x,
                                                               double* __restrict__ npart, double* __restrict__ tpart,
                                                               int64_t ldp, int32_t part_rank, int32_t part_count,
                                                               uint32_t ncached, FinArgs f, int32_t fin_pending,
                                                               const Ctrl* __restrict__ ctrl,
                                                               const double* __restrict__ scales) {
  asm volatile("" ::"s"(M), "s"(n), "s"(npart), "s"(tpart), "s"(ldp), "s"(part_rank), "s"(part_count), "s"(ncached),
               "s"(fin_pending), "s"(ctrl));
  if (COMPACT) asm volatile("" ::"s"(scales));
  if (ctrl->stop) return;
  if (blockIdx.x == 0) {
    if (fin_pending) finalize_body<false, kWave>(f);
    return;
  }
  symv_lower_body<true, COMPACT>(blockIdx.x - 1u, 0u, M, n, 0, x, npart, tpart, ldp, part_rank, part_count, ncached,
                                 scales);
}

__global__ __launch_bounds__(kWave) void symv_lower_batch_kernel(const double* const* __restrict__ Ms, int64_t n,
                                                                 const double* __restrict__ x0, int64_t xstride,
                                                                 double* __restrict__ npart0,
                                                                 double* __restrict__ tpart0, int64_t pstride,
                                                                 int64_t ldp, uint32_t ncached, FinArgs f,
                                                                 int32_t fin_pending, const Ctrl* __restrict__ ctrl) {
  asm volatile("" ::"s"(Ms), "s"(n), "s"(xstride), "s"(npart0), "s"(tpart0), "s"(pstride), "s"(ldp), "s"(ncached),
               "s"(fin_pending), "s"(ctrl));
  if (ctrl && ctrl->stop) return;
  if (blockIdx.x == 0) {
    if (blockIdx.y == 0 && fin_pending) finalize_body<false, kWave>(f);
    return;
  }
  const int64_t k = blockIdx.y;
  symv_lower_body<true>(blockIdx.x - 1u, 0u, Ms[k], n, 0, x0 + k * xstride, npart0 + k * pstride, tpart0 + k * pstride,
                        ldp, 0, 1, ncached);
}

__global__ __launch_bounds__(kBlock) void symv_reduce_kernel(const double* __restrict__ npart,
                                                             const double* __restrict__ tpart, int64_t ldp,
                                                             int64_t n, int32_t ntile, double* __restrict__ y,
                                                             const Ctrl* __restrict__ ctrl) {
  if (ctrl && ctrl->stop) return;
  const int slot = threadIdx.x >> 4;
  const int64_t i = static_cast<int64_t>(blockIdx.x) * 16 + (threadIdx.x & 15);
  double s = 0.0;
  if (i < n) {
    const int32_t d = static_cast<int32_t>(i / kTile);
#pragma unroll 4
    for (int32_t p = slot; p <= ntile; p += 16) {
      const double* src = (p <= d) ? npart + static_cast<int64_t>(p) * ldp : tpart + static_cast<int64_t>(p - 1) * ldp;
      s += src[i];
    }
  }
  fold_slots_store(s, y, i, i < n);
}

__global__ __launch_bounds__(kBlock) void symv_small_kernel(const double* __restrict__ M, int64_t n, int64_t ld,
                                                            const double* __restrict__ x, double* __restrict__ y,
                                                            const Ctrl* __restrict__ ctrl) {
  if (ctrl && ctrl->stop) return;
  const int lane = threadIdx.x & 63, wid = threadIdx.x >> 6;
  const int64_t j = static_cast<int64_t>(blockIdx.x) * 4 + wid;
  if (j >= n) return;
  const double* __restrict__ col = M + j * ld;
  const int64_t npairs = n >> 1;
  double a0 = 0.0, a1 = 0.0;
  for (int64_t p = lane; p < npairs; p += 64) {
    const double2_t m2 = *reinterpret_cast<const double2_t*>(col + 2 * p);
    const double2_t x2 = *reinterpret_cast<const double2_t*>(x + 2 * p);
    a0 = __builtin_fma(m2.x, x2.x, a0);
    a1 = __builtin_fma(m2.y, x2.y, a1);
  }
  double s = a0 + a1;
  if ((n & 1) && lane == 0) s = __builtin_fma(col[n - 1], x[n - 1], s);
  s = wave_sum(s);
  if (lane == 0) y[j] = s;
}

void launch_symv_small(const double* M, int64_t n, int64_t ld, const double* x, double* y, const Ctrl* ctrl,
                       hipStream_t stream) {
  hipLaunchKernelGGL(symv_small_kernel, dim3(static_cast<unsigned>(ceil_div(n, 4))), dim3(kBlock), 0, stream, M, n,
                     ld, x, y, ctrl);
}

__device__ __forceinline__ int64_t cq_quantise(double v, int shift) {
  const double lim = 140737488355327.0;
  double q = rint(ldexp(v, shift));
  q = q > lim ? lim : (q < -lim ? -lim : q);
  return static_cast<int64_t>(q);
}

__global__ __launch_bounds__(kBlock) void symv_compact_pack_kernel(const double* __restrict__ M, int64_t ld, int packed,
                                                                   char* __restrict__ C, double* __restrict__ scales,
                                                                   double* __restrict__ deq) {
  __shared__ double wmax[kBlock / kWave];
  const unsigned t = blockIdx.x;
  unsigned bi, bj;
  tri_decode(t, bi, bj);
  const int64_t sld = packed ? kTile : ld;
  const double* src = packed ? M + static_cast<int64_t>(t) * (kTile * kTile)
                             : M + static_cast<int64_t>(bj) * kTile * ld + static_cast<int64_t>(bi) * kTile;
  char* dst = C + cq_tile_offset(t, bi);
  double* dq = deq ? deq + static_cast<int64_t>(t) * (kTile * kTile) : nullptr;
  if (bi == bj) {
    for (int e = 2 * threadIdx.x; e < kTile * kTile; e += 2 * kBlock) {
      const double2_t v = *reinterpret_cast<const double2_t*>(src + static_cast<int64_t>(e / kTile) * sld + (e % kTile));
      *reinterpret_cast<double2_t*>(reinterpret_cast<double*>(dst) + e) = v;
      if (dq) *reinterpret_cast<double2_t*>(dq + e) = v;
    }
    if (threadIdx.x == 0) scales[t] = 1.0;
    return;
  }
  double mx = 0.0;
  for (int e = 2 * threadIdx.x; e < kTile * kTile; e += 2 * kBlock) {
    const double2_t v = *reinterpret_cast<const double2_t*>(src + static_cast<int64_t>(e / kTile) * sld + (e % kTile));
    mx = fmax(mx, fmax(fabs(v.x), fabs(v.y)));
  }
  mx = wave_max(mx);
  if ((threadIdx.x & 63) == 0) wmax[threadIdx.x >> 6] = mx;
  __syncthreads();
  mx = fmax(fmax(wmax[0], wmax[1]), fmax(wmax[2], wmax[3]));
  int ex = 0;
  if (mx > 0.0) (void)frexp(mx, &ex);
  const int shift = kCqBits - 1 - ex;
  const double scale = mx > 0.0 ? ldexp(1.0, -shift) : 0.0;
  if (threadIdx.x == 0) scales[t] = scale;
  constexpr int kRuns = 3 * kWave;
  for (int c = threadIdx.x; c < (kTile / kSyPanel) * kRuns; c += kBlock) {
    const int p = c / kRuns, run = (c % kRuns) / kWave, l = c % kWave, r = 2 * l;
    uint4_t out;
    if (run < 2) {
#pragma unroll
      for (int k = 0; k < 2; ++k) {
        const int col = kSyPanel * p + 2 * run + k;
        const double2_t v = *reinterpret_cast<const double2_t*>(src + col * sld + r);
        const int64_t q0 = cq_quantise(v.x, shift), q1 = cq_quantise(v.y, shift);
        out[2 * k] = static_cast<unsigned>(q0 & 0xffffffff);
        out[2 * k + 1] = static_cast<unsigned>(q1 & 0xffffffff);
        if (dq) *reinterpret_cast<double2_t*>(dq + col * kTile + r) =
            double2_t{static_cast<double>(q0) * scale, static_cast<double>(q1) * scale};
      }
    } else {
#pragma unroll
      for (int k = 0; k < kSyPanel; ++k) {
        const double2_t v = *reinterpret_cast<const double2_t*>(src + (kSyPanel * p + k) * sld + r);
        const int64_t q0 = cq_quantise(v.x, shift), q1 = cq_quantise(v.y, shift);
        out[k] = (static_cast<unsigned>(q0 >> 32) & 0xffffu) | (static_cast<unsigned>(q1 >> 32) << 16);
      }
    }
    *reinterpret_cast<uint4_t*>(dst + p * kCqPanelBytes + run * 1024 + l * 16) = out;
  }
}

SymvPlan symv_plan(int64_t n) {
  SymvPlan p{};
  p.n = n;
  p.npad = round_up(n, kTile);
  p.ldp = p.npad;
  p.ntile = static_cast<int32_t>(p.npad / kTile);
  p.packed = false;
  p.compact = false;
  p.scales = nullptr;
  p.ncached = symv_cached_tiles(p, kSymvCacheBytes);
  return p;
}

int64_t symv_tiles(const SymvPlan& p) { return static_cast<int64_t>(p.ntile) * (p.ntile + 1) / 2; }
size_t symv_packed_elems(const SymvPlan& p) { return static_cast<size_t>(symv_tiles(p)) * kTile * kTile; }

int64_t symv_tile_prefix_bytes(const SymvPlan& p, int64_t t) {
  if (!p.compact) return t * int64_t{8} * kTile * kTile;
  unsigned bi, bj;
  tri_decode(static_cast<unsigned>(t), bi, bj);
  return cq_tile_offset(static_cast<unsigned>(t), bi);
}
size_t symv_compact_elems(const SymvPlan& p) {
  SymvPlan c = p;
  c.compact = true;
  return static_cast<size_t>(symv_tile_prefix_bytes(c, symv_tiles(p)) / 8 + symv_tiles(p));
}
double* symv_compact_scales(const SymvPlan& p, double* C) {
  SymvPlan c = p;
  c.compact = true;
  return C + symv_tile_prefix_bytes(c, symv_tiles(p)) / 8;
}

int64_t symv_cached_tiles(const SymvPlan& p, int64_t budget_bytes) {
  const int64_t tiles = symv_tiles(p);
  if (!stream_hint(symv_tile_prefix_bytes(p, tiles))) return tiles;
  if (!p.compact) return std::min(tiles, budget_bytes / (int64_t{8} * kTile * kTile));
  int64_t lo = 0, hi = tiles;
  while (lo < hi) {
    const int64_t mid = (lo + hi + 1) / 2;
    if (symv_tile_prefix_bytes(p, mid) <= budget_bytes) lo = mid;
    else hi = mid - 1;
  }
  return lo;
}

void launch_symv_pack(const SymvPlan& p, const double* M, int64_t ld, double* P, hipStream_t stream) {
  launch_tri_pack(M, ld, P, static_cast<unsigned>(symv_tiles(p)), 0, stream);
}

void launch_symv_compact_pack(const SymvPlan& p, const double* M, int64_t ld, bool src_packed, double* C, double* deq,
                              hipStream_t stream) {
  hipLaunchKernelGGL(symv_compact_pack_kernel, dim3(static_cast<unsigned>(symv_tiles(p))), dim3(kBlock), 0, stream, M,
                     ld, src_packed ? 1 : 0, reinterpret_cast<char*>(C), symv_compact_scales(p, C), deq);
}

void launch_symv_reduce(const SymvPlan& p, const double* npart, const double* tpart, double* y, const Ctrl* ctrl,
                        hipStream_t stream) {
  hipLaunchKernelGGL(symv_reduce_kernel, dim3(static_cast<unsigned>(ceil_div(p.n, 16))), dim3(kBlock), 0, stream, npart,
                     tpart, p.ldp, p.n, p.ntile, y, ctrl);
}

void launch_symv_lower(const SymvPlan& p, const double* M, int64_t ld, const double* x, double* npart, double* tpart,
                       double* y, const Ctrl* ctrl, hipStream_t stream, int part_rank, int part_count, bool reduce) {
  const uint32_t ncached = static_cast<uint32_t>(p.ncached < 0 ? 0 : p.ncached);
  const double* none = nullptr;
  if (p.packed && p.compact)
    hipLaunchKernelGGL((symv_lower_kernel<true, true>), dim3(static_cast<unsigned>(symv_tiles(p))), dim3(kWave), 0,
                       stream, M, p.n, ld, x, npart, tpart, p.ldp, part_rank, part_count, ncached, ctrl, p.scales);
  else if (p.packed)
    hipLaunchKernelGGL(symv_lower_kernel<true>, dim3(static_cast<unsigned>(symv_tiles(p))), dim3(kWave), 0, stream, M,
                       p.n, ld, x, npart, tpart, p.ldp, part_rank, part_count, ncached, ctrl, none);
  else
    hipLaunchKernelGGL(symv_lower_kernel<false>, dim3(static_cast<unsigned>(p.ntile), static_cast<unsigned>(p.ntile)),
                       dim3(kWave), 0, stream, M, p.n, ld, x, npart, tpart, p.ldp, part_rank, part_count, ncached,
                       ctrl, none);
  if (reduce) launch_symv_reduce(p, npart, tpart, y, ctrl, stream);
}

void launch_symv_lower_batch(const SymvPlan& p, const double* const* Ms_dev, int32_t K, const double* x0, int64_t xstride,
                             double* npart0, double* tpart0, int64_t pstride, const Ctrl* ctrl, hipStream_t stream,
                             const FinArgs* fin) {
  const uint32_t ncached = static_cast<uint32_t>(p.ncached < 0 ? 0 : p.ncached);
  const FinArgs f = fin ? *fin : FinArgs{};
  const dim3 grid(static_cast<unsigned>(symv_tiles(p)) + 1u, static_cast<unsigned>(K));
  hipLaunchKernelGGL(symv_lower_batch_kernel, grid, dim3(kWave), 0, stream, Ms_dev, p.n, x0, xstride, npart0, tpart0,
                     pstride, p.ldp, ncached, f, fin ? 1 : 0, ctrl);
}

void launch_symv_lower_fin(const SymvPlan& p, const double* M, const double* x, double* npart, double* tpart,
                           const FinArgs& f, bool fin_pending, const Ctrl* ctrl, hipStream_t stream, int part_rank,
                           int part_count, double* y) {
  const uint32_t ncached = static_cast<uint32_t>(p.ncached < 0 ? 0 : p.ncached);
  const dim3 grid(static_cast<unsigned>(symv_tiles(p)) + 1u);
  const double* none = nullptr;
  if (p.compact)
    hipLaunchKernelGGL(symv_lower_fin_kernel<true>, grid, dim3(kWave), 0, stream, M, p.n, x, npart, tpart, p.ldp,
                       part_rank, part_count, ncached, f, fin_pending ? 1 : 0, ctrl, p.scales);
  else
    hipLaunchKernelGGL(symv_lower_fin_kernel<false>, grid, dim3(kWave), 0, stream, M, p.n, x, npart, tpart, p.ldp,
                       part_rank, part_count, ncached, f, fin_pending ? 1 : 0, ctrl, none);
  if (y) launch_symv_reduce(p, npart, tpart, y, ctrl, stream);
}

}
```

admm-project_amd/csrc/tri_tile.h:

```cpp
#pragma once
#include "wave_reduce.h"

namespace admm {

typedef double double2_t __attribute__((ext_vector_type(2)));

constexpr int kTile = 128;

__host__ __device__ __forceinline__ void tri_decode(unsigned t, unsigned& bi, unsigned& bj) {
  unsigned r = static_cast<unsigned>((sqrt(8.0 * t + 1.0) - 1.0) * 0.5);
  while (r * (r + 1u) / 2u > t) --r;
  while ((r + 1u) * (r + 2u) / 2u <= t) ++r;
  bi = r;
  bj = t - r * (r + 1u) / 2u;
}

constexpr int64_t kCqUnit = 32768;
constexpr int kCqPanelBytes = 3 * 1024;
constexpr int kCqBits = 48;
__host__ __device__ __forceinline__ int64_t cq_tile_offset(unsigned t, unsigned bi) {
  return (int64_t{3} * t + bi) * kCqUnit;
}

__device__ __forceinline__ double readlane_f64(double v, int l) {
  const int lo = __builtin_amdgcn_readlane(__double2loint(v), l);
  const int hi = __builtin_amdgcn_readlane(__double2hiint(v), l);
  return __hiloint2double(hi, lo);
}

template <int P, bool NT>
__device__ __forceinline__ void panel_load(const double* __restrict__ Mr, int64_t ld, int64_t c, double2_t (&d)[P]) {
#pragma unroll
  for (int k = 0; k < P; ++k) d[k] = load2<NT>(Mr + (c + k) * ld);
}

template <int P>
__device__ __forceinline__ void panel_fma(double2_t pair, int co, const double2_t (&d)[P], double& a0, double& a1) {
#pragma unroll
  for (int k = 0; k < P; ++k) {
    const double xj = readlane_f64((k & 1) ? pair.y : pair.x, (co + k) >> 1);
    a0 = __builtin_fma(d[k].x, xj, a0);
    a1 = __builtin_fma(d[k].y, xj, a1);
  }
}

struct SyLane {
  const double* M;
  const double* x;
  int64_t ld, n;
  int r;
  double xr0, xr1;
};

template <bool NT>
__device__ __forceinline__ void sy_load(const SyLane& s, int64_t cp, double2_t (&d)[kSyPanel]) {
#pragma unroll
  for (int k = 0; k < kSyPanel; ++k) d[k] = load2<NT>(s.M + (cp + k) * s.ld + s.r);
}

template <bool NT>
struct SyBuf64 {
  double2_t d[kSyPanel];
  __device__ __forceinline__ void load(const SyLane& s, int64_t cp) { sy_load<NT>(s, cp, d); }
  __device__ __forceinline__ void get(double2_t (&o)[kSyPanel]) const {
#pragma unroll
    for (int k = 0; k < kSyPanel; ++k) o[k] = d[k];
  }
};

typedef unsigned uint4_t __attribute__((ext_vector_type(4)));
template <bool NT>
__device__ __forceinline__ uint4_t load16(const char* p) {
  const uint4_t* q = reinterpret_cast<const uint4_t*>(p);
  return NT ? __builtin_nontemporal_load(q) : *q;
}
__device__ __forceinline__ double cq_value(unsigned lo, int hi) {
  return __builtin_fma(static_cast<double>(hi), 4294967296.0, static_cast<double>(lo));
}
template <bool NT>
struct SyBufCq {
  uint4_t lo[2], hi;
  __device__ __forceinline__ void load(const SyLane& s, int64_t cp) {
    const char* p = reinterpret_cast<const char*>(s.M) + (cp >> 2) * kCqPanelBytes + s.r * 8;
    lo[0] = load16<NT>(p);
    lo[1] = load16<NT>(p + 1024);
    hi = load16<NT>(p + 2048);
  }
  __device__ __forceinline__ void get(double2_t (&o)[kSyPanel]) const {
#pragma unroll
    for (int k = 0; k < kSyPanel; ++k) {
      const int h = static_cast<int>(hi[k]);
      o[k].x = cq_value(lo[k >> 1][2 * (k & 1)], static_cast<int>(static_cast<short>(h)));
      o[k].y = cq_value(lo[k >> 1][2 * (k & 1) + 1], h >> 16);
    }
  }
};

template <bool DIAG, bool NP = true, bool TP = true>
__device__ __forceinline__ void sy_compute(const SyLane& s, int64_t cp, const double2_t (&d)[kSyPanel], double& n0,
                                           double& n1, double* __restrict__ tout, int lane) {
  double tacc[kSyPanel];
#pragma unroll
  for (int k = 0; k < kSyPanel; ++k) {
    const int64_t j = cp + k;
    const double xj = NP ? s.x[j < s.n ? j : s.n - 1] : 0.0;
    double a0 = d[k].x, a1 = d[k].y;
    double t0 = a0, t1 = a1;
    if (DIAG) {
      t0 = (s.r > j) ? a0 : 0.0;
      t1 = (s.r + 1 > j) ? a1 : 0.0;
      a0 = (j <= s.r) ? a0 : 0.0;
      a1 = (j <= s.r + 1) ? a1 : 0.0;
    }
    if (TP) tacc[k] = __builtin_fma(t0, s.xr0, t1 * s.xr1);
    if (NP) {
      n0 = __builtin_fma(a0, xj, n0);
      n1 = __builtin_fma(a1, xj, n1);
    }
  }
  if (TP) {
    const double sum = reduce_scatter4(tacc);
    if ((lane & 15) == 0) tout[cp + (lane >> 4)] = sum;
  }
}

template <bool DIAG, class BUF, bool NP, bool TP, int NBUF>
__device__ __forceinline__ void sy_tile_ring(const SyLane& s, int64_t c0, double& n0, double& n1,
                                             double* __restrict__ tout, int lane) {
  constexpr int kPanels = kTile / kSyPanel, kFull = (kPanels / NBUF) * NBUF;
  static_assert(NBUF >= 2 && NBUF <= 8, "ring of panel buffers");
  BUF buf[NBUF];
  double2_t d[kSyPanel];
#pragma unroll
  for (int b = 0; b + 1 < NBUF; ++b) buf[b].load(s, c0 + b * kSyPanel);
#pragma unroll 1
  for (int g = 0; g < kFull; g += NBUF) {
#pragma unroll
    for (int b = 0; b < NBUF; ++b) {
      const int nxt = g + b + NBUF - 1;
      if (kFull - NBUF + b + NBUF - 1 < kPanels || nxt < kPanels)
        buf[(b + NBUF - 1) % NBUF].load(s, c0 + nxt * kSyPanel);
      buf[b].get(d);
      sy_compute<DIAG, NP, TP>(s, c0 + (g + b) * kSyPanel, d, n0, n1, tout, lane);
    }
  }
#pragma unroll
  for (int b = 0; b < kPanels - kFull; ++b) {
    if (kFull + b + NBUF - 1 < kPanels) buf[(b + NBUF - 1) % NBUF].load(s, c0 + (kFull + b + NBUF - 1) * kSyPanel);
    buf[b].get(d);
    sy_compute<DIAG, NP, TP>(s, c0 + (kFull + b) * kSyPanel, d, n0, n1, tout, lane);
  }
}

template <bool DIAG, bool NT, bool NP = true, bool TP = true, int NBUF = 2>
__device__ __forceinline__ void sy_tile(const SyLane& s, int64_t c0, double& n0, double& n1,
                                        double* __restrict__ tout, int lane) {
  sy_tile_ring<DIAG, SyBuf64<NT>, NP, TP, NBUF>(s, c0, n0, n1, tout, lane);
}

template <bool NT, int NBUF = 2>
__device__ __forceinline__ void sy_tile_cq(SyLane& s, double scale, double& n0, double& n1, double* __restrict__ tout,
                                           int lane) {
  s.xr0 *= scale;
  s.xr1 *= scale;
  sy_tile_ring<false, SyBufCq<NT>, true, true, NBUF>(s, 0, n0, n1, tout, lane);
  n0 *= scale;
  n1 *= scale;
}

}
```

admm-project_amd/engine.py:

```python
from __future__ import annotations

import ctypes as C

import numpy as np

from . import _lib as L

_STOPCOND = {"standard": L.STOP_STANDARD, "hnorm": L.STOP_HNORM, "both": L.STOP_BOTH, "none": L.STOP_NONE}


def _f64(a, order="F"):
    return np.require(np.asarray(a, dtype=np.float64), dtype=np.float64, requirements=[order, "A"])


def _weights(w, count, what, name="weights"):
    if w is None:
        return None
    w = np.ascontiguousarray(np.asarray(w, dtype=np.float64).reshape(-1))
    if w.size != count:
        raise ValueError(f"{name} has {w.size} entries for {count} {what}")
    return w


class Engine:
# ... 365 lines not shown
        else:
            Bm = np.asfortranarray(np.asarray(B, dtype=np.float64))
            L.check(self._lib.admm_engine_set_constraint_b(self._h, L.as_dp(Bm), Bm.shape[0], Bm.shape[1], L.MEM_HOST,
                                                           0.0, none, None))
            self.nB = int(Bm.shape[1])

    def set_groups(self, sizes=None, weights=None):
        if sizes is None:
            L.check(self._lib.admm_engine_set_groups(self._h, None, 0, None))
            return
        g = np.ascontiguousarray(np.asarray(sizes, dtype=np.int64).reshape(-1))
        w = None if weights is None else np.ascontiguousarray(np.asarray(weights, dtype=np.float64).reshape(-1))
        if w is not None and w.size != g.size:
            raise ValueError(f"weights has {w.size} entries for {g.size} groups")
        L.check(self._lib.admm_engine_set_groups(self._h, g.ctypes.data_as(C.POINTER(C.c_int64)), g.size,
                                                 None if w is None else L.as_dp(w)))

    def set_tv2d_isotropic(self, on=True):
        L.check(self._lib.admm_engine_set_tv2d_isotropic(self._h, int(on)))

    def set_penalty(self, l1weights=None, ridge=0.0, nonnegative=0, l1=0.0):
        if l1weights is None and ridge == 0.0 and nonnegative == 0 and l1 == 0.0:
            L.check(self._lib.admm_engine_set_penalty(self._h, None))
            return
        w = _weights(l1weights, self.nB, "coefficients", "l1weights")
        d = L.PenaltyDesc(None if w is None else L.as_dp(w), float(l1), float(ridge), int(nonnegative))
        L.check(self._lib.admm_engine_set_penalty(self._h, C.byref(d)))

    def penalty(self):
        d, has = L.PenaltyDesc(), C.c_int32()
        L.check(self._lib.admm_engine_get_penalty(self._h, C.byref(d), C.byref(has)))
        return dict(l1=d.l1, ridge=d.ridge, nonnegative=int(d.nonnegative), has_l1weights=bool(has.value))

    def set_loss(self, weights=None, slopes=(1.0, 1.0), epsilon=0.0, delta=1.0):
        a, b = (float(v) for v in slopes)
        if weights is None and a == 1.0 and b == 1.0 and epsilon == 0.0 and delta == 1.0:
            L.check(self._lib.admm_engine_set_loss(self._h, None))
            return
        w = _weights(weights, self.nB, "observations")
        d = L.LossDesc(None if w is None else L.as_dp(w), a, b, float(epsilon), float(delta))
        L.check(self._lib.admm_engine_set_loss(self._h, C.byref(d)))

    def loss(self):
        d, has = L.LossDesc(), C.c_int32()
        L.check(self._lib.admm_engine_get_loss(self._h, C.byref(d), C.byref(has)))
        return dict(slopes=(d.slope_pos, d.slope_neg), epsilon=d.epsilon, delta=d.delta, has_weights=bool(has.value))

    def set_svm_cost(self, weights=None, classcost=(1.0, 1.0)):
        cp, cn = (float(v) for v in classcost)
        if weights is None and cp == 1.0 and cn == 1.0:
            L.check(self._lib.admm_engine_set_svm_cost(self._h, None))
            return
        w = _weights(weights, self.nB, "observations")
        d = L.SvmCostDesc(None if w is None else L.as_dp(w), cp, cn)
        L.check(self._lib.admm_engine_set_svm_cost(self._h, C.byref(d)))

    def svm_cost(self):
        d, has = L.SvmCostDesc(), C.c_int32()
        L.check(self._lib.admm_engine_get_svm_cost(self._h, C.byref(d), C.byref(has)))
        return dict(classcost=(d.cost_pos, d.cost_neg), has_weights=bool(has.value))

    def close(self):
        if getattr(self, "_h", None):
            self._lib.admm_engine_destroy(self._h)
            self._h = None

    def __del__(self):
        try:
            self.close()
        except Exception:
            pass

    @property
    def setup_seconds(self):
        v = C.c_double(0)
        L.check(self._lib.admm_engine_setup_seconds(self._h, C.byref(v)))
        return v.value

    def xsolve_storage(self):
        form, nbytes = C.c_int32(), C.c_int64()
        ea, eb, diff = C.c_double(), C.c_double(), C.c_double()
        L.check(self._lib.admm_engine_xsolve_storage(self._h, C.byref(form), C.byref(nbytes), C.byref(ea), C.byref(eb),
                                                     C.byref(diff)))
        return dict(form="compact" if form.value == L.STORAGE_COMPACT else "fp64", stored_bytes=nbytes.value,
                    probe_err_compact=ea.value, probe_err_fp64=eb.value, probe_diff=diff.value)

    def info(self):
        i = L.EngineInfo()
        i.struct_size = C.sizeof(L.EngineInfo)
        L.check(self._lib.admm_engine_info(self._h, C.byref(i)))
        names = {L.XSOLVE_AUTO: "auto", L.XSOLVE_TRSV: "trsv", L.XSOLVE_INVERSE: "inverse", L.XSOLVE_CG: "cg",
                 L.XSOLVE_CALLBACK: "callback", L.XSOLVE_PINV: "pinv"}
        return dict(xsolve_requested=names.get(i.xsolve_requested, i.xsolve_requested),
                    xsolve_used=names.get(i.xsolve_used, i.xsolve_used), pinv_used=bool(i.pinv_used),
                    probed=bool(i.probed), unwrapped_fused=bool(i.unwrapped_fused), trsv_blocks=i.trsv_blocks, jacobi_sweeps=i.jacobi_sweeps,
                    factor_n=i.factor_n, rank=i.rank, cond_estimate=i.cond_estimate,
                    probe_err_inverse=i.probe_err_inverse, probe_err_trsv=i.probe_err_trsv, probe_err_trsv_one=i.probe_err_trsv_one, probe_diff=i.probe_diff,
                    xsolve_cacheable_bytes=i.xsolve_cacheable_bytes, xsolve_stream_bytes=i.xsolve_stream_bytes,
                    obj_bound_max=i.obj_bound_max, obj_form_literal=bool(i.obj_form_literal), ngroups=i.ngroups)

    def sparse_info(self):
        if not getattr(self, "sparse", False):
            return None
        v = self.fetch(L.F_SPARSE_NNZ, 3)
        return dict(nnz=int(v[0]), lanes=(int(v[1]), int(v[2])))

    def set_profiling(self, on, stride=1):
        L.check(self._lib.admm_engine_set_profiling_stride(self._h, int(stride)))
        if on is True:
            mask = -1
        elif not on:
            mask = 0
        else:
            mask = 0
            for k in on:
                mask |= 1 << int(k)
        L.check(self._lib.admm_engine_set_profiling(self._h, mask))

    def kernel_time(self, which):
        ms, cnt = C.c_double(0), C.c_int64(0)
        L.check(self._lib.admm_engine_kernel_time(self._h, which, C.byref(ms), C.byref(cnt)))
        return ms.value, cnt.value

    def run(self, *, rho=1.0, maxiters=1000, domaxiters=0, relax=1.0, fast=L.FAST_OFF, objevals=0, convtest=0,
            convtol=1e-10, stopcond="standard", nodualerror=0, abstol=1e-5, reltol=1e-3, Hnormtol=1e-6,
            restart=0.999, dvaltol=1e-8, record_history=1, check_every=0, x0=None, z0=None, u0=None,
            stale_factor_ok=0):
        keep = []
        o = self._options(keep, rho=rho, maxiters=maxiters, domaxiters=domaxiters, relax=relax, fast=fast,
                          objevals=objevals, convtest=convtest, convtol=convtol, stopcond=stopcond,
                          nodualerror=nodualerror, abstol=abstol, reltol=reltol, Hnormtol=Hnormtol, restart=restart,
                          dvaltol=dvaltol, record_history=record_history, check_every=check_every, x0=x0, z0=z0, u0=u0,
                          stale_factor_ok=stale_factor_ok)
        s = L.RunSummary()
        self._cb_error = None
        rc = self._lib.admm_engine_run(self._h, C.byref(o), C.byref(s))
        if rc != L.OK and self._cb_error is not None:
            exc, self._cb_error = self._cb_error, None
            raise exc
        L.check(rc)
        self.last = s
        return s

    def _options(self, keep, *, rho=1.0, maxiters=1000, domaxiters=0, relax=1.0, fast=L.FAST_OFF, objevals=0,
                 convtest=0, convtol=1e-10, stopcond="standard", nodualerror=0, abstol=1e-5, reltol=1e-3,
                 Hnormtol=1e-6, restart=0.999, dvaltol=1e-8, record_history=1, check_every=0, x0=None, z0=None,
                 u0=None, stale_factor_ok=0):
        o = L.Options()
        self._lib.admm_options_default(C.byref(o))
        o.rho, o.relax, o.abstol, o.reltol = float(rho), float(relax), float(abstol), float(reltol)
        o.Hnormtol, o.convtol, o.restart, o.dvaltol = float(Hnormtol), float(convtol), float(restart), float(dvaltol)
        o.maxiters = int(maxiters)
        o.domaxiters = int(bool(domaxiters))
        o.fast = int(fast)
        o.objevals = int(bool(objevals))
        o.convtest = int(bool(convtest))
        o.stopcond = _STOPCOND[stopcond]
        o.nodualerror = int(bool(nodualerror))
        o.record_history = int(bool(record_history))
        o.check_every = int(check_every)
        o.stale_factor_ok = int(bool(stale_factor_ok))
        for name, val in (("x0", x0), ("z0", z0), ("u0", u0)):
            if val is not None:
                a = _f64(val).reshape(-1)
                keep.append(a)
                setattr(o, name, L.as_dp(a))
        self._relax = float(relax)
# ... 189 lines not shown
```

include/admm_engine.h:

```cpp
#ifndef ADMM_ENGINE_H
#define ADMM_ENGINE_H

#include <stddef.h>
#include <stdint.h>

#ifdef __cplusplus
extern "C" {
#endif

#define ADMM_ABI_VERSION 5

enum {
  ADMM_OK = 0,
  ADMM_E_INVALID = -1,
  ADMM_E_UNSUPPORTED = -2,
  ADMM_E_DEVICE = -3,
  ADMM_E_NUMERIC = -4,
  ADMM_E_COMM = -5,
  ADMM_E_CAPACITY = -6
};

enum {
  ADMM_PROB_LASSO = 1,
  ADMM_PROB_LASSO_CONSENSUS = 2,
// ... 134 lines not shown
  ADMM_F_CONS_U = 22,
  ADMM_F_WVALS = 23,
  ADMM_F_COVSEL_S = 24,
  ADMM_F_TV2D_ROW_STAGE = 25,
  ADMM_F_SPARSE_NNZ = 26
};

int admm_abi_version(void);
const char* admm_last_error(void);
int admm_device_count(int* count);
int admm_device_info(int device, char* name, size_t cap, int64_t* hbm_bytes, int32_t* cus);

void admm_options_default(admm_options* opts);
void admm_problem_desc_default(admm_problem_desc* desc);
int admm_engine_create(const admm_problem_desc* desc, admm_engine** out);
typedef struct admm_sparse_desc {
  int32_t struct_size;
  int32_t mem;
  int64_t rows, cols, nnz;
  const double* val;
  const uint64_t* ir;
  const uint64_t* jc;
} admm_sparse_desc;
int admm_engine_create_sparse(const admm_problem_desc* desc, const admm_sparse_desc* D, admm_engine** out);
int admm_engine_set_callbacks(admm_engine* eng, admm_prox_callback xmin, void* xuser, admm_prox_callback zmin,
                              void* zuser, admm_obj_callback obj, void* objuser);
int admm_engine_set_operators(admm_engine* eng, admm_operator_callback A, void* Auser, admm_operator_callback At,
                              void* Atuser);
int admm_engine_set_hooks(admm_engine* eng, admm_altu_callback altu, void* altu_user, admm_norms_callback norms,
                          void* norms_user);
int admm_engine_set_constraint_b(admm_engine* eng, const double* B, int64_t ldB, int64_t nB, int32_t memkind,
                                 double scalar, admm_operator_callback Bop, void* Buser);
int admm_engine_set_groups(admm_engine* eng, const int64_t* sizes, int32_t ngroups, const double* weights);
typedef struct admm_penalty_desc {
  const double* l1weights;
  double l1;
  double ridge;
  int32_t nonnegative;
} admm_penalty_desc;
int admm_engine_set_penalty(admm_engine* eng, const admm_penalty_desc* desc);
int admm_engine_get_penalty(admm_engine* eng, admm_penalty_desc* desc, int32_t* has_l1weights);
typedef struct admm_loss_desc {
  const double* weights;
  double slope_pos;
  double slope_neg;
  double epsilon;
  double delta;
} admm_loss_desc;
int admm_engine_set_loss(admm_engine* eng, const admm_loss_desc* desc);
int admm_engine_get_loss(admm_engine* eng, admm_loss_desc* desc, int32_t* has_weights);
typedef struct admm_svm_cost_desc {
  const double* weights;
  double cost_pos;
  double cost_neg;
} admm_svm_cost_desc;
int admm_engine_set_svm_cost(admm_engine* eng, const admm_svm_cost_desc* desc);
int admm_engine_get_svm_cost(admm_engine* eng, admm_svm_cost_desc* desc, int32_t* has_weights);
int admm_engine_set_tv2d_isotropic(admm_engine* eng, int32_t on);
int admm_engine_run(admm_engine* eng, const admm_options* opts, admm_run_summary* summary);
int admm_engine_fetch(admm_engine* eng, int field, double* dst, size_t cap, size_t* written);
typedef struct admm_engine_info_t {
  int32_t struct_size;
  int32_t xsolve_requested;
  int32_t xsolve_used;
  int32_t pinv_used;
  int32_t probed;
  int32_t trsv_blocks;
  int32_t jacobi_sweeps;
  int32_t unwrapped_fused;
  int64_t factor_n;
  int64_t rank;
  double cond_estimate;
  double probe_err_inverse;
  double probe_err_trsv;
  double probe_diff;
  int64_t xsolve_cacheable_bytes;
  int64_t xsolve_stream_bytes;
  double obj_bound_max;
  int32_t obj_form_literal;
  int32_t ngroups;
  double probe_err_trsv_one;
} admm_engine_info_t;
int admm_engine_info(admm_engine* eng, admm_engine_info_t* info);
enum { ADMM_STORAGE_FP64 = 0, ADMM_STORAGE_COMPACT = 1 };
int admm_engine_xsolve_storage(admm_engine* eng, int32_t* form, int64_t* stored_bytes, double* probe_err_compact,
                               double* probe_err_fp64, double* probe_diff);
int admm_xsolve_compact_accept(double err_compact, double err_fp64, double diff);
enum { ADMM_TV2D_ROWS_AUTO = 0, ADMM_TV2D_ROWS_GREEN = 1, ADMM_TV2D_ROWS_COOP = 2, ADMM_TV2D_ROWS_DCT = 3,
       ADMM_TV2D_ROWS_THOMAS = 4 };
int admm_tv2d_row_stage(int64_t H, int64_t W, double rho);
int admm_tv2d_rows_green_taps(double rho);
int admm_dct_tables(int64_t n, double* tw, double* c4, double* lam, double* chirp, double* hbr, int64_t counts[5]);
int admm_engine_setup_seconds(admm_engine* eng, double* seconds);
enum { ADMM_K_XSOLVE = 0, ADMM_K_GEMV_N = 1, ADMM_K_GEMV_T = 2, ADMM_K_PROX = 3, ADMM_K_FINALIZE = 4, ADMM_K_COUNT = 5 };
int admm_engine_kernel_time(admm_engine* eng, int which, double* total_ms, int64_t* launches);
int admm_engine_set_profiling(admm_engine* eng, int mask);
int admm_engine_set_profiling_stride(admm_engine* eng, int stride);
void admm_engine_destroy(admm_engine* eng);

enum { ADMM_FIELD_NUMERIC = 0,
       ADMM_FIELD_TEXT = 1,
       ADMM_FIELD_HANDLE = 2,
       ADMM_FIELD_SPARSE = 3,
       ADMM_FIELD_OTHER = 4 };
typedef struct admm_field {
  const char* name;
  int32_t kind;
  int32_t reserved;
  const double* data;
  int64_t rows, cols;
  const char* text;
  const uint64_t* ir;
  const uint64_t* jc;
} admm_field;
typedef struct admm_binding admm_binding;
int admm_binding_create(const char* problem, const admm_field* args, int32_t nargs, const admm_field* handles,
                        int32_t nhandles, admm_binding** out);
void admm_binding_destroy(admm_binding* b);
const admm_problem_desc* admm_binding_desc(const admm_binding* b);
typedef struct admm_binding_info {
  int32_t struct_size;
  int32_t problem;
  int64_t nA, nB, nU;
  int32_t a_handle;
  int32_t b_kind;
  double b_scalar;
  const double* b_matrix;
  int64_t b_ld;
} admm_binding_info;
int admm_binding_get_info(const admm_binding* b, admm_binding_info* info);
const admm_sparse_desc* admm_binding_sparse(const admm_binding* b);
int admm_binding_apply(const admm_binding* b, admm_engine* eng);
int admm_binding_options(const admm_binding* b, const admm_field* options, int32_t nopt, const admm_field* handles,
                         int32_t nhandles, admm_options* out);
enum { ADMM_RES_FETCH = 0,
       ADMM_RES_SCALAR = 1,
       ADMM_RES_START = 2 };
typedef struct admm_result_field {
  const char* name;
  int32_t kind, source;
  int64_t rows, cols;
  double scalar;
} admm_result_field;
int admm_binding_results(admm_binding* b, const admm_options* opts, const admm_run_summary* summary,
                         admm_result_field* out, int32_t cap, int32_t* count);

int admm_memcpy_d2h(void* host_dst, const void* device_src, size_t bytes, void* hip_stream);
int admm_memcpy_h2d(void* device_dst, const void* host_src, size_t bytes, void* hip_stream);

int admm_op_gemv_n(const double* D, int64_t m, int64_t n, int64_t ldD, const double* x, double* y);
int admm_op_gemv_t(const double* D, int64_t m, int64_t n, int64_t ldD, const double* V, int64_t ldV,
                   int32_t nrhs, double* G, int64_t ldG);
int admm_op_spmv(const admm_sparse_desc* D, int transpose, const double* x, double* y);
int admm_op_spmm(const admm_sparse_desc* D, int transpose, int K, const double* X, double* Y);
int admm_op_spmm_weighted(const admm_sparse_desc* D, int32_t K, const double* X, const double* obsweights, int32_t nfolds,
                          const int32_t* fold, const int32_t* heldout, double* Y);
int admm_op_spmm_cg(const admm_sparse_desc* D, int32_t K, const double* Y, const double* X0, double shift, double tol,
                    int32_t maxit, int32_t batch, const int32_t* stop, double* X, double* R, int64_t* state,
                    int32_t* next_batch);
int admm_op_gram(const double* D, int64_t m, int64_t n, int64_t ldD, double shift, double* W);
int admm_op_cholesky(double* A, int64_t n, int64_t ldA);
int admm_op_trsv_pair(const double* L, int64_t n, int64_t ldL, const double* y, double* x);
int admm_op_soft_threshold(const double* v, int64_t n, double t, double* out);
int admm_op_group_soft_threshold(const double* v, int64_t n, const int64_t* sizes, int32_t ngroups,
                                 const double* weights, double lambda_over_rho, double* out);
int admm_op_penalty_prox(const double* v, int64_t n, const int64_t* sizes, int32_t ngroups, const double* groupweights,
                         double lambda_over_rho, const admm_penalty_desc* desc, double rho, double* out);
int admm_op_loss_prox(const double* v, int64_t len, int32_t problem, const admm_loss_desc* desc, double rho, double* out);
int admm_op_svm_prox(const double* v, const double* ell, int64_t len, int32_t loss, double C, double rho,
                     const admm_svm_cost_desc* desc, double* out);
int admm_op_pair_soft_threshold(const double* v, int64_t N, double t, double* out);
int admm_op_symv(const double* M, int64_t n, int64_t ldM, const double* x, int32_t form, int64_t ncached,
                 int32_t part_count, double* y);
int admm_op_symv_compact(const double* M, int64_t n, int64_t ldM, const double* x, int32_t fin, int64_t ncached,
                         int32_t part_count, double* y, double* Q, int64_t ldQ);
int admm_op_symv_batch(const double* Ms, int64_t n, int64_t ldM, int32_t K, const double* X, int64_t ldX,
                       int64_t ncached, double* Y, int64_t ldY);
int admm_op_gemm(int32_t transA, int32_t transB, int64_t M, int64_t N, int64_t K, double alpha, const double* A,
                 int64_t lda, const double* B, int64_t ldb, double beta, double* C, int64_t ldc, int32_t lower_only);
int admm_op_trtri(const double* L, int64_t n, int64_t ldL, double* X, int64_t ldX);
int admm_op_llt_apply(const double* L, int64_t n, int64_t ldL, const double* x, double* y);
int admm_op_dct_cols(const double* img, int64_t H, int64_t W, int32_t inverse, double* out);
int admm_op_tv2d_rows(const double* src, int64_t H, int64_t W, double rho, int32_t form, double* out);
int admm_op_tv2d_xsolve(const double* b, int64_t H, int64_t W, double rho, int32_t form, double* x);
int admm_op_consensus_tail(int32_t form, int64_t n, int32_t K, int32_t Ntot, double rho, double lambda,
                           const double* rows, double* X, double* U, const double* Dts, double* xave, double* ubar,
                           const double* remote, int32_t with_q, double* Y, double* sums, double* z, double* xaveprev,
                           double* slots, double* q);

#define ADMM_COMM_ID_BYTES 128
enum { ADMM_COMM_RCCL = 0, ADMM_COMM_SHM = 1,
       ADMM_COMM_P2P = 2 };
int admm_comm_unique_id(char id[ADMM_COMM_ID_BYTES]);
int admm_comm_init(const char id[ADMM_COMM_ID_BYTES], int rank, int nranks, int device, int transport,
                   admm_comm** out);
int admm_comm_info(admm_comm* comm, int* rank, int* nranks, int* transport);
int admm_comm_allreduce_sum(admm_comm* comm, double* host_buf, size_t count);
int admm_comm_measure_latency(admm_comm* comm, size_t count, int reps, double* microseconds);
void admm_comm_destroy(admm_comm* comm);

int admm_comm_init_all(int nranks, const int* devices, int transport, admm_comm** comms);
int admm_engine_create_all(int nranks, const admm_problem_desc* descs, admm_engine** engines);
int admm_engine_run_all(int nranks, admm_engine* const* engines, const admm_options* opts, int opts_per_rank,
                        admm_run_summary* summaries);

typedef struct admm_svm_ovr admm_svm_ovr;
#define ADMM_SVM_OVR_MAX_N 448

typedef struct admm_svm_ovr_desc {
  int32_t struct_size;
  int32_t K;
  int64_t m, n;
  const double* D;
  int64_t ldD;
  const double* ELL;
  const int32_t* loss;
  double C;
  int32_t mem;
  int32_t device;
  const double* Dplus;
  admm_comm* comm;
} admm_svm_ovr_desc;

typedef struct admm_svm_ovr_options {
  int32_t struct_size;
  int32_t maxiters;
  double rho;
  double abstol;
  double reltol;
  double Hnormtol;
  double relax;
  int32_t fast;
  int32_t convtest;
  int32_t domaxiters;
  int32_t objevals;
  int32_t check_every;
  int32_t reserved0;
  const double* x0;
  const double* z0;
  const double* u0;
} admm_svm_ovr_options;

typedef struct admm_svm_ovr_summary {
  int32_t steps;
  int32_t stopped_early;
  double objopt;
} admm_svm_ovr_summary;

enum {
  ADMM_OVR_F_XOPT = 1,
  ADMM_OVR_F_ZOPT = 2,
  ADMM_OVR_F_UOPT = 3,
  ADMM_OVR_F_PNORM = 4, ADMM_OVR_F_PERR = 5, ADMM_OVR_F_HNORMSQ = 6, ADMM_OVR_F_OBJEVALS = 7
};

void admm_svm_ovr_desc_default(admm_svm_ovr_desc* desc);
void admm_svm_ovr_options_default(admm_svm_ovr_options* opts);
int admm_svm_ovr_create(const admm_svm_ovr_desc* desc, admm_svm_ovr** out);
// ... 529 lines not shown
```

Measured before the change: 17480 iterations/s.

## Add 40-bit compact storage for the cached inverse factor in symv

Adds a 40-bit fixed-point tile format alongside the existing 48-bit compact storage for the packed inverse matrix used in the x-update symv. When the 48-bit form would exceed the cache budget, the engine first tries 40-bit storage and keeps it if it passes the accuracy probe, otherwise it falls back to 48-bit. This reduces the bytes streamed per iteration and lets more tiles fit in cache. The cost is coarser quantisation, which the accuracy check may reject, plus slightly more bit-unpacking work per element.

```diff
diff --git a/admm-project_amd/_lib.py b/admm-project_amd/_lib.py
--- a/admm-project_amd/_lib.py
+++ b/admm-project_amd/_lib.py
@@ -360,7 +360,7 @@
 
 FIELD_NUMERIC, FIELD_TEXT, FIELD_HANDLE, FIELD_SPARSE, FIELD_OTHER = 0, 1, 2, 3, 4
 RES_FETCH, RES_SCALAR, RES_START = 0, 1, 2
-STORAGE_FP64, STORAGE_COMPACT = 0, 1
+STORAGE_FP64, STORAGE_COMPACT, STORAGE_COMPACT40 = 0, 1, 2
 F_WVALS = 23
 F_COVSEL_S = 24
 F_TV2D_ROW_STAGE = 25
@@ -441,6 +441,8 @@
     "admm_op_symv": (C.c_int, [_dp, C.c_int64, C.c_int64, _dp, C.c_int32, C.c_int64, C.c_int32, _dp]),
     "admm_op_symv_compact": (C.c_int, [_dp, C.c_int64, C.c_int64, _dp, C.c_int32, C.c_int64, C.c_int32, _dp, _dp,
                                        C.c_int64]),
+    "admm_op_symv_compact_bits": (C.c_int, [_dp, C.c_int64, C.c_int64, _dp, C.c_int32, C.c_int64, C.c_int32, _dp, _dp,
+                                            C.c_int64, C.c_int32]),
     "admm_op_symv_batch": (C.c_int, [_dp, C.c_int64, C.c_int64, C.c_int32, _dp, C.c_int64, C.c_int64, _dp, C.c_int64]),
     "admm_op_gemm": (C.c_int, [C.c_int32, C.c_int32, C.c_int64, C.c_int64, C.c_int64, C.c_double, _dp, C.c_int64, _dp,
                                C.c_int64, C.c_double, _dp, C.c_int64, C.c_int32]),
diff --git a/admm-project_amd/csrc/dev/symv_packed.hip b/admm-project_amd/csrc/dev/symv_packed.hip
--- a/admm-project_amd/csrc/dev/symv_packed.hip
+++ b/admm-project_amd/csrc/dev/symv_packed.hip
@@ -368,33 +368,44 @@
     last_us = us;
     printf("%-44s %8.2f us  %6.3f TB/s\n", name, us, ntri * 131072.0 / us * 1e-6);
   };
-  if (argc > 2 && std::string(argv[2]) == "compact") {
-    SymvPlan pf = p, pc = p;
-    pf.packed = pc.packed = pc.compact = true;
-    double* C;
-    CK(hipMalloc(&C, sizeof(double) * symv_compact_elems(pc)));
-    launch_symv_compact_pack(pc, P, 0, true, C, nullptr, 0);
-    pc.scales = symv_compact_scales(pc, C);
+  const std::string mode = argc > 2 ? argv[2] : "";
+  if (mode == "compact" || mode == "compact40") {
+    const bool c40 = mode == "compact40";
+    SymvPlan pf = p, pc[2] = {p, p};
+    pf.packed = true;
+    double* C[2] = {nullptr, nullptr};
+    double cmb[2] = {0.0, 0.0};
+    const int nform = c40 ? 2 : 1;
+    for (int k = 0; k < nform; ++k) {
+      pc[k].packed = true;
+      pc[k].cbits = k ? 40 : 48;
+      CK(hipMalloc(&C[k], sizeof(double) * symv_compact_elems(pc[k])));
+      launch_symv_compact_pack(pc[k], P, 0, true, C[k], nullptr, 0);
+      pc[k].scales = symv_compact_scales(pc[k], C[k]);
+      cmb[k] = symv_tile_prefix_bytes(pc[k], ntri) * 1e-6;
+      printf("compact storage, %d bits: %.1f MB (TB/s column: fp64 algorithmic bytes over time)\n", pc[k].cbits, cmb[k]);
+    }
     CK(hipDeviceSynchronize());
-    const double cmb = symv_tile_prefix_bytes(pc, ntri) * 1e-6;
-    printf("compact storage %.1f MB (TB/s column: fp64 algorithmic bytes over time)\n", cmb);
     std::vector<double> h1(n), h2(n);
     for (int round = 0; round < 2; ++round)
       for (int64_t mb : {0, 64, 105, 136, 168, 200, 232, 264, 290, 320}) {
         char nm[96];
         pf.ncached = symv_cached_tiles(pf, mb << 20);
-        pc.ncached = symv_cached_tiles(pc, mb << 20);
-        snprintf(nm, sizeof nm, "fp64    %3lld MB cacheable (%lld tiles)", (long long)mb, (long long)pf.ncached);
+        snprintf(nm, sizeof nm, "fp64      %3lld MB cacheable (%lld tiles)", (long long)mb, (long long)pf.ncached);
         time_it(nm, [&] { launch_symv_lower(pf, P, 0, x, np_, tp, y, nullptr, 0, 0, 1, false); }, y);
-        snprintf(nm, sizeof nm, "compact %3lld MB cacheable (%lld tiles)", (long long)mb, (long long)pc.ncached);
-        time_it(nm, [&] { launch_symv_lower(pc, C, 0, x, np_, tp, y2, nullptr, 0, 0, 1, false); }, y2);
-        printf("   compact over stored bytes: %6.3f TB/s\n", cmb / last_us);
+        for (int k = 0; k < nform; ++k) {
+          pc[k].ncached = symv_cached_tiles(pc[k], mb << 20);
+          snprintf(nm, sizeof nm, "compact%s %3lld MB cacheable (%lld tiles)", k ? "40" : "  ", (long long)mb,
+                   (long long)pc[k].ncached);
+          time_it(nm, [&] { launch_symv_lower(pc[k], C[k], 0, x, np_, tp, y2, nullptr, 0, 0, 1, false); }, y2);
+          printf("   compact%s over stored bytes: %6.3f TB/s\n", k ? "40" : "", cmb[k] / last_us);
+        }
       }
     CK(hipMemcpy(h1.data(), y, sizeof(double) * n, hipMemcpyDeviceToHost));
     CK(hipMemcpy(h2.data(), y2, sizeof(double) * n, hipMemcpyDeviceToHost));
     double err = 0, ymax = 0;
     for (int64_t i = 0; i < n; ++i) err = fmax(err, fabs(h1[i] - h2[i])), ymax = fmax(ymax, fabs(h1[i]));
-    printf("max |y_compact - y_fp64| / max |y| = %.3e\n", err / ymax);
+    printf("max |y_%s - y_fp64| / max |y| = %.3e\n", c40 ? "compact40" : "compact", err / ymax);
     return 0;
   }
   time_it("column-major padded (production)", [&] {
diff --git a/admm-project_amd/csrc/engine.hip b/admm-project_amd/csrc/engine.hip
--- a/admm-project_amd/csrc/engine.hip
+++ b/admm-project_amd/csrc/engine.hip
@@ -327,13 +327,23 @@
   return err_compact <= std::max(1e-11, 4.0 * err_fp64) && diff <= std::max(1e-11, 8.0 * err_fp64);
 }
 
+static int try_symv_storage(admm_engine* e, SliceFactor& f, int bits, bool* kept);
 static int choose_symv_storage(admm_engine* e, SliceFactor& f) {
-  if (f.mode != ADMM_XSOLVE_INVERSE || !f.Minv || !f.F || f.pinv || !f.planSy.packed || f.planSy.compact ||
+  if (f.mode != ADMM_XSOLVE_INVERSE || !f.Minv || !f.F || f.pinv || !f.planSy.packed || f.planSy.cbits ||
       f.n < kSymvHalfMin || e->sy_split || e->keep_fp64)
     return ADMM_OK;
   if (!stream_hint(symv_tile_prefix_bytes(f.planSy, symv_tiles(f.planSy)))) return ADMM_OK;
+  SymvPlan c48 = f.planSy;
+  c48.cbits = 48;
+  bool kept = false;
+  if (symv_tile_prefix_bytes(c48, symv_tiles(c48)) > kSymvCacheBytes) ADMM_TRY(try_symv_storage(e, f, 40, &kept));
+  if (!kept) ADMM_TRY(try_symv_storage(e, f, 48, &kept));
+  return ADMM_OK;
+}
+
+static int try_symv_storage(admm_engine* e, SliceFactor& f, int bits, bool* kept) {
   SymvPlan cp = f.planSy;
-  cp.compact = true;
+  cp.cbits = bits;
   double* C = nullptr;
   ADMM_TRY(e->mem.alloc(&C, symv_compact_elems(cp)));
   launch_symv_compact_pack(cp, f.Minv, 0, true, C, nullptr, e->stream);
@@ -350,7 +360,8 @@
   f.err_cq = ea;
   f.err_cq_ref = eb;
   f.cq_diff = diff;
-  if (symv_compact_accept(ea, eb, diff)) {
+  *kept = symv_compact_accept(ea, eb, diff);
+  if (*kept) {
     e->mem.free_one(f.Minv);
     f.Minv = C;
     f.planSy = cp;
@@ -934,7 +945,8 @@
   if (!e) return fail(ADMM_E_INVALID, "engine is NULL");
   const SliceFactor& f = e->xfac;
   const bool inv = f.mode == ADMM_XSOLVE_INVERSE && f.Minv;
-  if (form) *form = (inv && f.planSy.compact) ? ADMM_STORAGE_COMPACT : ADMM_STORAGE_FP64;
+  if (form)
+    *form = !(inv && f.planSy.cbits) ? ADMM_STORAGE_FP64 : f.planSy.cbits == 40 ? ADMM_STORAGE_COMPACT40 : ADMM_STORAGE_COMPACT;
   if (stored_bytes) {
     *stored_bytes = 0;
     if (inv && f.planSy.packed) *stored_bytes = symv_tile_prefix_bytes(f.planSy, symv_tiles(f.planSy));
diff --git a/admm-project_amd/csrc/kernels.h b/admm-project_amd/csrc/kernels.h
--- a/admm-project_amd/csrc/kernels.h
+++ b/admm-project_amd/csrc/kernels.h
@@ -37,7 +37,7 @@
   int32_t ntile;
   bool packed;
   int64_t ncached;
-  bool compact;
+  int32_t cbits;
   const double* scales;
   size_t npart_elems() const { return static_cast<size_t>(ntile) * ldp; }
   size_t tpart_elems() const { return static_cast<size_t>(ntile) * ldp; }
diff --git a/admm-project_amd/csrc/l1class.hip b/admm-project_amd/csrc/l1class.hip
--- a/admm-project_amd/csrc/l1class.hip
+++ b/admm-project_amd/csrc/l1class.hip
@@ -437,7 +437,7 @@
   }
   const SliceFactor& f = e->xfac;
   const size_t kp = static_cast<size_t>(o->Kp);
-  if (f.mode == ADMM_XSOLVE_INVERSE && f.Minv && !f.pinv && !f.planSy.compact) {
+  if (f.mode == ADMM_XSOLVE_INVERSE && f.Minv && !f.pinv && !f.planSy.cbits) {
     o->plan = f.planSy;
     if (f.planSy.packed) {
       o->P = f.Minv;
diff --git a/admm-project_amd/csrc/lasso_multi.hip b/admm-project_amd/csrc/lasso_multi.hip
--- a/admm-project_amd/csrc/lasso_multi.hip
+++ b/admm-project_amd/csrc/lasso_multi.hip
@@ -116,7 +116,7 @@
   o->ldt = round_up(n, 2);
   const SliceFactor& f = e->xfac;
   const size_t kp = static_cast<size_t>(o->chunks) * KC;
-  if (f.mode == ADMM_XSOLVE_INVERSE && f.Minv && !f.pinv && !f.planSy.compact) {
+  if (f.mode == ADMM_XSOLVE_INVERSE && f.Minv && !f.pinv && !f.planSy.cbits) {
     o->plan = f.planSy;
     if (f.planSy.packed) {
       o->P = f.Minv;
diff --git a/admm-project_amd/csrc/ops.hip b/admm-project_amd/csrc/ops.hip
--- a/admm-project_amd/csrc/ops.hip
+++ b/admm-project_amd/csrc/ops.hip
@@ -517,8 +517,14 @@
 
 int admm_op_symv_compact(const double* M, int64_t n, int64_t ldM, const double* x, int32_t fin, int64_t ncached,
                          int32_t part_count, double* y, double* Q, int64_t ldQ) {
+  return admm_op_symv_compact_bits(M, n, ldM, x, fin, ncached, part_count, y, Q, ldQ, 48);
+}
+
+int admm_op_symv_compact_bits(const double* M, int64_t n, int64_t ldM, const double* x, int32_t fin, int64_t ncached,
+                              int32_t part_count, double* y, double* Q, int64_t ldQ, int32_t bits) {
   if (!M || !x || !y || n <= 0 || ldM < n || ncached < -1 || part_count < 1 || (Q && ldQ < n))
     return fail(ADMM_E_INVALID, "symv_compact: bad argument (ncached >= -1, part_count >= 1, ldQ >= n)");
+  if (bits != 40 && bits != 48) return fail(ADMM_E_INVALID, "symv_compact: the compact tile widths are 40 and 48 bits");
   ADMM_TRY(need_device());
   Scratch sc;
   double *dM, *dx, *dy, *dC, *dQ = nullptr, *npart, *tpart;
@@ -526,7 +532,8 @@
   ADMM_TRY(sc.alloc(&dy, round_up(n, 2)));
   ADMM_HIP_TRY(hipMemcpy(dx, x, sizeof(double) * n, hipMemcpyHostToDevice));
   SymvPlan plan = symv_plan(n);
-  plan.packed = plan.compact = true;
+  plan.packed = true;
+  plan.cbits = bits;
   ADMM_TRY(sc.alloc(&dM, static_cast<size_t>(plan.npad) * plan.npad));
   ADMM_HIP_TRY(hipMemset(dM, 0, sizeof(double) * plan.npad * plan.npad));
   ADMM_TRY(put_padded(dM, plan.npad, M, n, ldM));
diff --git a/admm-project_amd/csrc/symv.hip b/admm-project_amd/csrc/symv.hip
--- a/admm-project_amd/csrc/symv.hip
+++ b/admm-project_amd/csrc/symv.hip
@@ -8,13 +8,15 @@
 
 namespace admm {
 
-template <bool PACKED, bool COMPACT = false, int NBUF = 2>
+template <bool PACKED, int CBITS = 0, int NBUF = 2>
 __device__ __forceinline__ void symv_lower_body(unsigned block_x, unsigned block_y, const double* __restrict__ M,
                                                 int64_t n, int64_t ld, const double* __restrict__ x,
                                                 double* __restrict__ npart, double* __restrict__ tpart, int64_t ldp,
                                                 int32_t part_rank, int32_t part_count, uint32_t ncached,
                                                 const double* __restrict__ scales = nullptr) {
-  static_assert(PACKED || !COMPACT, "the compact storage is tile-packed");
+  static_assert(PACKED || !CBITS, "the compact storage is tile-packed");
+  constexpr bool COMPACT = CBITS != 0;
+  constexpr int BITS = COMPACT ? CBITS : 48;
   unsigned bi, bj, lin;
   if (PACKED) {
     lin = block_x;
@@ -34,7 +36,7 @@
   int64_t cbase;
   double* __restrict__ tout = tpart + static_cast<int64_t>(bi) * ldp;
   if (PACKED) {
-    s.M = COMPACT ? reinterpret_cast<const double*>(reinterpret_cast<const char*>(M) + cq_tile_offset(lin, bi))
+    s.M = COMPACT ? reinterpret_cast<const double*>(reinterpret_cast<const char*>(M) + cq_tile_offset<BITS>(lin, bi))
                   : M + static_cast<int64_t>(lin) * (kTile * kTile);
     s.x = x + c0;
     s.ld = kTile;
@@ -55,17 +57,17 @@
   double n0 = 0.0, n1 = 0.0;
   if (lin < ncached) {
     if (bi == bj) sy_tile<true, false, true, true, NBUF>(s, cbase, n0, n1, tout, lane);
-    else if (COMPACT) sy_tile_cq<false, NBUF>(s, scales[lin], n0, n1, tout, lane);
+    else if (COMPACT) sy_tile_cq<false, BITS, NBUF>(s, scales[lin], n0, n1, tout, lane);
     else sy_tile<false, false, true, true, NBUF>(s, cbase, n0, n1, tout, lane);
   } else {
     if (bi == bj) sy_tile<true, true, true, true, NBUF>(s, cbase, n0, n1, tout, lane);
-    else if (COMPACT) sy_tile_cq<true, NBUF>(s, scales[lin], n0, n1, tout, lane);
+    else if (COMPACT) sy_tile_cq<true, BITS, NBUF>(s, scales[lin], n0, n1, tout, lane);
     else sy_tile<false, true, true, true, NBUF>(s, cbase, n0, n1, tout, lane);
   }
   *reinterpret_cast<double2_t*>(npart + static_cast<int64_t>(bj) * ldp + gr) = double2_t{n0, n1};
 }
 
-template <bool PACKED, bool COMPACT = false>
+template <bool PACKED, int CBITS = 0>
 __global__ __launch_bounds__(kWave) void symv_lower_kernel(const double* __restrict__ M, int64_t n, int64_t ld,
                                                            const double* __restrict__ x, double* __restrict__ npart,
                                                            double* __restrict__ tpart, int64_t ldp,
@@ -73,11 +75,11 @@
                                                            const Ctrl* __restrict__ ctrl,
                                                            const double* __restrict__ scales) {
   if (ctrl && ctrl->stop) return;
-  symv_lower_body<PACKED, COMPACT>(blockIdx.x, blockIdx.y, M, n, ld, x, npart, tpart, ldp, part_rank, part_count,
+  symv_lower_body<PACKED, CBITS>(blockIdx.x, blockIdx.y, M, n, ld, x, npart, tpart, ldp, part_rank, part_count,
                                    ncached, scales);
 }
 
-template <bool COMPACT>
+template <int CBITS>
 __global__ __launch_bounds__(kWave) void symv_lower_fin_kernel(const double* __restrict__ M, int64_t n,
                                                                const double* __restrict__ x,
                                                                double* __restrict__ npart, double* __restrict__ tpart,
@@ -87,13 +89,13 @@
                                                                const double* __restrict__ scales) {
   asm volatile("" ::"s"(M), "s"(n), "s"(npart), "s"(tpart), "s"(ldp), "s"(part_rank), "s"(part_count), "s"(ncached),
                "s"(fin_pending), "s"(ctrl));
-  if (COMPACT) asm volatile("" ::"s"(scales));
+  if (CBITS) asm volatile("" ::"s"(scales));
   if (ctrl->stop) return;
   if (blockIdx.x == 0) {
     if (fin_pending) finalize_body<false, kWave>(f);
     return;
   }
-  symv_lower_body<true, COMPACT>(blockIdx.x - 1u, 0u, M, n, 0, x, npart, tpart, ldp, part_rank, part_count, ncached,
+  symv_lower_body<true, CBITS>(blockIdx.x - 1u, 0u, M, n, 0, x, npart, tpart, ldp, part_rank, part_count, ncached,
                                  scales);
 }
 
@@ -162,13 +164,15 @@
                      ld, x, y, ctrl);
 }
 
+template <int BITS>
 __device__ __forceinline__ int64_t cq_quantise(double v, int shift) {
-  const double lim = 140737488355327.0;
+  constexpr double lim = static_cast<double>((int64_t{1} << (BITS - 1)) - 1);
   double q = rint(ldexp(v, shift));
   q = q > lim ? lim : (q < -lim ? -lim : q);
   return static_cast<int64_t>(q);
 }
 
+template <int BITS>
 __global__ __launch_bounds__(kBlock) void symv_compact_pack_kernel(const double* __restrict__ M, int64_t ld, int packed,
                                                                    char* __restrict__ C, double* __restrict__ scales,
                                                                    double* __restrict__ deq) {
@@ -179,7 +183,8 @@
   const int64_t sld = packed ? kTile : ld;
   const double* src = packed ? M + static_cast<int64_t>(t) * (kTile * kTile)
                              : M + static_cast<int64_t>(bj) * kTile * ld + static_cast<int64_t>(bi) * kTile;
-  char* dst = C + cq_tile_offset(t, bi);
+  typedef CqFormat<BITS> F;
+  char* dst = C + cq_tile_offset<BITS>(t, bi);
   double* dq = deq ? deq + static_cast<int64_t>(t) * (kTile * kTile) : nullptr;
   if (bi == bj) {
     for (int e = 2 * threadIdx.x; e < kTile * kTile; e += 2 * kBlock) {
@@ -201,33 +206,39 @@
   mx = fmax(fmax(wmax[0], wmax[1]), fmax(wmax[2], wmax[3]));
   int ex = 0;
   if (mx > 0.0) (void)frexp(mx, &ex);
-  const int shift = kCqBits - 1 - ex;
+  const int shift = BITS - 1 - ex;
   const double scale = mx > 0.0 ? ldexp(1.0, -shift) : 0.0;
   if (threadIdx.x == 0) scales[t] = scale;
   constexpr int kRuns = 3 * kWave;
   for (int c = threadIdx.x; c < (kTile / kSyPanel) * kRuns; c += kBlock) {
     const int p = c / kRuns, run = (c % kRuns) / kWave, l = c % kWave, r = 2 * l;
-    uint4_t out;
+    char* rec = dst + p * F::kPanelBytes + run * 1024;
     if (run < 2) {
+      uint4_t out;
 #pragma unroll
       for (int k = 0; k < 2; ++k) {
         const int col = kSyPanel * p + 2 * run + k;
         const double2_t v = *reinterpret_cast<const double2_t*>(src + col * sld + r);
-        const int64_t q0 = cq_quantise(v.x, shift), q1 = cq_quantise(v.y, shift);
+        const int64_t q0 = cq_quantise<BITS>(v.x, shift), q1 = cq_quantise<BITS>(v.y, shift);
         out[2 * k] = static_cast<unsigned>(q0 & 0xffffffff);
         out[2 * k + 1] = static_cast<unsigned>(q1 & 0xffffffff);
         if (dq) *reinterpret_cast<double2_t*>(dq + col * kTile + r) =
             double2_t{static_cast<double>(q0) * scale, static_cast<double>(q1) * scale};
       }
+      *reinterpret_cast<uint4_t*>(rec + l * 16) = out;
     } else {
+      uintn_t<F::kHiDwords> out = {};
+      constexpr unsigned mask = (1u << F::kHiBits) - 1u;
 #pragma unroll
       for (int k = 0; k < kSyPanel; ++k) {
         const double2_t v = *reinterpret_cast<const double2_t*>(src + (kSyPanel * p + k) * sld + r);
-        const int64_t q0 = cq_quantise(v.x, shift), q1 = cq_quantise(v.y, shift);
-        out[k] = (static_cast<unsigned>(q0 >> 32) & 0xffffu) | (static_cast<unsigned>(q1 >> 32) << 16);
+        const int64_t q0 = cq_quantise<BITS>(v.x, shift), q1 = cq_quantise<BITS>(v.y, shift);
+        const int bit = 2 * k * F::kHiBits;
+        out[bit / 32] |= ((static_cast<unsigned>(q0 >> 32) & mask) << (bit % 32)) |
+                         ((static_cast<unsigned>(q1 >> 32) & mask) << (bit % 32 + F::kHiBits));
       }
+      *reinterpret_cast<uintn_t<F::kHiDwords>*>(rec + l * (4 * F::kHiDwords)) = out;
     }
-    *reinterpret_cast<uint4_t*>(dst + p * kCqPanelBytes + run * 1024 + l * 16) = out;
   }
 }
 
@@ -238,7 +249,7 @@
   p.ldp = p.npad;
   p.ntile = static_cast<int32_t>(p.npad / kTile);
   p.packed = false;
-  p.compact = false;
+  p.cbits = 0;
   p.scales = nullptr;
   p.ncached = symv_cached_tiles(p, kSymvCacheBytes);
   return p;
@@ -248,26 +259,20 @@
 size_t symv_packed_elems(const SymvPlan& p) { return static_cast<size_t>(symv_tiles(p)) * kTile * kTile; }
 
 int64_t symv_tile_prefix_bytes(const SymvPlan& p, int64_t t) {
-  if (!p.compact) return t * int64_t{8} * kTile * kTile;
+  if (!p.cbits) return t * int64_t{8} * kTile * kTile;
   unsigned bi, bj;
   tri_decode(static_cast<unsigned>(t), bi, bj);
-  return cq_tile_offset(static_cast<unsigned>(t), bi);
+  return p.cbits == 40 ? cq_tile_offset<40>(static_cast<unsigned>(t), bi) : cq_tile_offset<48>(static_cast<unsigned>(t), bi);
 }
 size_t symv_compact_elems(const SymvPlan& p) {
-  SymvPlan c = p;
-  c.compact = true;
-  return static_cast<size_t>(symv_tile_prefix_bytes(c, symv_tiles(p)) / 8 + symv_tiles(p));
-}
-double* symv_compact_scales(const SymvPlan& p, double* C) {
-  SymvPlan c = p;
-  c.compact = true;
-  return C + symv_tile_prefix_bytes(c, symv_tiles(p)) / 8;
-}
+  return static_cast<size_t>(symv_tile_prefix_bytes(p, symv_tiles(p)) / 8 + symv_tiles(p));
+}
+double* symv_compact_scales(const SymvPlan& p, double* C) { return C + symv_tile_prefix_bytes(p, symv_tiles(p)) / 8; }
 
 int64_t symv_cached_tiles(const SymvPlan& p, int64_t budget_bytes) {
   const int64_t tiles = symv_tiles(p);
   if (!stream_hint(symv_tile_prefix_bytes(p, tiles))) return tiles;
-  if (!p.compact) return std::min(tiles, budget_bytes / (int64_t{8} * kTile * kTile));
+  if (!p.cbits) return std::min(tiles, budget_bytes / (int64_t{8} * kTile * kTile));
   int64_t lo = 0, hi = tiles;
   while (lo < hi) {
     const int64_t mid = (lo + hi + 1) / 2;
@@ -283,8 +288,13 @@
 
 void launch_symv_compact_pack(const SymvPlan& p, const double* M, int64_t ld, bool src_packed, double* C, double* deq,
                               hipStream_t stream) {
-  hipLaunchKernelGGL(symv_compact_pack_kernel, dim3(static_cast<unsigned>(symv_tiles(p))), dim3(kBlock), 0, stream, M,
-                     ld, src_packed ? 1 : 0, reinterpret_cast<char*>(C), symv_compact_scales(p, C), deq);
+  const dim3 grid(static_cast<unsigned>(symv_tiles(p)));
+  if (p.cbits == 40)
+    hipLaunchKernelGGL(symv_compact_pack_kernel<40>, grid, dim3(kBlock), 0, stream, M, ld, src_packed ? 1 : 0,
+                       reinterpret_cast<char*>(C), symv_compact_scales(p, C), deq);
+  else
+    hipLaunchKernelGGL(symv_compact_pack_kernel<48>, grid, dim3(kBlock), 0, stream, M, ld, src_packed ? 1 : 0,
+                       reinterpret_cast<char*>(C), symv_compact_scales(p, C), deq);
 }
 
 void launch_symv_reduce(const SymvPlan& p, const double* npart, const double* tpart, double* y, const Ctrl* ctrl,
@@ -297,8 +307,11 @@
                        double* y, const Ctrl* ctrl, hipStream_t stream, int part_rank, int part_count, bool reduce) {
   const uint32_t ncached = static_cast<uint32_t>(p.ncached < 0 ? 0 : p.ncached);
   const double* none = nullptr;
-  if (p.packed && p.compact)
-    hipLaunchKernelGGL((symv_lower_kernel<true, true>), dim3(static_cast<unsigned>(symv_tiles(p))), dim3(kWave), 0,
+  if (p.packed && p.cbits == 40)
+    hipLaunchKernelGGL((symv_lower_kernel<true, 40>), dim3(static_cast<unsigned>(symv_tiles(p))), dim3(kWave), 0,
+                       stream, M, p.n, ld, x, npart, tpart, p.ldp, part_rank, part_count, ncached, ctrl, p.scales);
+  else if (p.packed && p.cbits)
+    hipLaunchKernelGGL((symv_lower_kernel<true, 48>), dim3(static_cast<unsigned>(symv_tiles(p))), dim3(kWave), 0,
                        stream, M, p.n, ld, x, npart, tpart, p.ldp, part_rank, part_count, ncached, ctrl, p.scales);
   else if (p.packed)
     hipLaunchKernelGGL(symv_lower_kernel<true>, dim3(static_cast<unsigned>(symv_tiles(p))), dim3(kWave), 0, stream, M,
@@ -326,11 +339,14 @@
   const uint32_t ncached = static_cast<uint32_t>(p.ncached < 0 ? 0 : p.ncached);
   const dim3 grid(static_cast<unsigned>(symv_tiles(p)) + 1u);
   const double* none = nullptr;
-  if (p.compact)
-    hipLaunchKernelGGL(symv_lower_fin_kernel<true>, grid, dim3(kWave), 0, stream, M, p.n, x, npart, tpart, p.ldp,
+  if (p.cbits == 40)
+    hipLaunchKernelGGL(symv_lower_fin_kernel<40>, grid, dim3(kWave), 0, stream, M, p.n, x, npart, tpart, p.ldp,
+                       part_rank, part_count, ncached, f, fin_pending ? 1 : 0, ctrl, p.scales);
+  else if (p.cbits)
+    hipLaunchKernelGGL(symv_lower_fin_kernel<48>, grid, dim3(kWave), 0, stream, M, p.n, x, npart, tpart, p.ldp,
                        part_rank, part_count, ncached, f, fin_pending ? 1 : 0, ctrl, p.scales);
   else
-    hipLaunchKernelGGL(symv_lower_fin_kernel<false>, grid, dim3(kWave), 0, stream, M, p.n, x, npart, tpart, p.ldp,
+    hipLaunchKernelGGL(symv_lower_fin_kernel<0>, grid, dim3(kWave), 0, stream, M, p.n, x, npart, tpart, p.ldp,
                        part_rank, part_count, ncached, f, fin_pending ? 1 : 0, ctrl, none);
   if (y) launch_symv_reduce(p, npart, tpart, y, ctrl, stream);
 }
diff --git a/admm-project_amd/csrc/tri_tile.h b/admm-project_amd/csrc/tri_tile.h
--- a/admm-project_amd/csrc/tri_tile.h
+++ b/admm-project_amd/csrc/tri_tile.h
@@ -15,11 +15,21 @@
   bj = t - r * (r + 1u) / 2u;
 }
 
-constexpr int64_t kCqUnit = 32768;
-constexpr int kCqPanelBytes = 3 * 1024;
-constexpr int kCqBits = 48;
+template <int BITS>
+struct CqFormat {
+  static_assert(BITS == 40 || BITS == 48, "compact tile widths");
+  static constexpr int kHiBits = BITS - 32;
+  static constexpr int kHiDwords = 8 * kHiBits / 32;
+  static constexpr int kPanelBytes = 2048 + 64 * 4 * kHiDwords;
+  static constexpr int64_t kUnit = (BITS == 48) ? 32768 : 16384;
+  static constexpr int kTileUnits = (kTile / 4) * kPanelBytes / kUnit;
+  static constexpr int kDiagUnits = 8 * kTile * kTile / kUnit;
+  static_assert(kTileUnits * kUnit == (kTile / 4) * kPanelBytes && kTileUnits == (BITS == 48 ? 3 : 5), "whole units");
+};
+template <int BITS>
 __host__ __device__ __forceinline__ int64_t cq_tile_offset(unsigned t, unsigned bi) {
-  return (int64_t{3} * t + bi) * kCqUnit;
+  typedef CqFormat<BITS> F;
+  return (int64_t{F::kTileUnits} * t + int64_t{F::kDiagUnits - F::kTileUnits} * bi) * F::kUnit;
 }
 
 __device__ __forceinline__ double readlane_f64(double v, int l) {
@@ -69,29 +79,36 @@
 };
 
 typedef unsigned uint4_t __attribute__((ext_vector_type(4)));
-template <bool NT>
-__device__ __forceinline__ uint4_t load16(const char* p) {
-  const uint4_t* q = reinterpret_cast<const uint4_t*>(p);
+template <int N>
+using uintn_t = unsigned __attribute__((ext_vector_type(N)));
+template <bool NT, int N>
+__device__ __forceinline__ uintn_t<N> loadn(const char* p) {
+  const uintn_t<N>* q = reinterpret_cast<const uintn_t<N>*>(p);
   return NT ? __builtin_nontemporal_load(q) : *q;
 }
 __device__ __forceinline__ double cq_value(unsigned lo, int hi) {
   return __builtin_fma(static_cast<double>(hi), 4294967296.0, static_cast<double>(lo));
 }
-template <bool NT>
+template <bool NT, int BITS>
 struct SyBufCq {
-  uint4_t lo[2], hi;
+  typedef CqFormat<BITS> F;
+  uint4_t lo[2];
+  uintn_t<F::kHiDwords> hi;
   __device__ __forceinline__ void load(const SyLane& s, int64_t cp) {
-    const char* p = reinterpret_cast<const char*>(s.M) + (cp >> 2) * kCqPanelBytes + s.r * 8;
-    lo[0] = load16<NT>(p);
-    lo[1] = load16<NT>(p + 1024);
-    hi = load16<NT>(p + 2048);
+    const char* p = reinterpret_cast<const char*>(s.M) + (cp >> 2) * F::kPanelBytes;
+    lo[0] = loadn<NT, 4>(p + s.r * 8);
+    lo[1] = loadn<NT, 4>(p + 1024 + s.r * 8);
+    hi = loadn<NT, F::kHiDwords>(p + 2048 + s.r * (2 * F::kHiDwords));
+  }
+  __device__ __forceinline__ int hi_field(int i) const {
+    const int bit = i * F::kHiBits;
+    return static_cast<int>(hi[bit / 32] << (32 - F::kHiBits - bit % 32)) >> (32 - F::kHiBits);
   }
   __device__ __forceinline__ void get(double2_t (&o)[kSyPanel]) const {
 #pragma unroll
     for (int k = 0; k < kSyPanel; ++k) {
-      const int h = static_cast<int>(hi[k]);
-      o[k].x = cq_value(lo[k >> 1][2 * (k & 1)], static_cast<int>(static_cast<short>(h)));
-      o[k].y = cq_value(lo[k >> 1][2 * (k & 1) + 1], h >> 16);
+      o[k].x = cq_value(lo[k >> 1][2 * (k & 1)], hi_field(2 * k));
+      o[k].y = cq_value(lo[k >> 1][2 * (k & 1) + 1], hi_field(2 * k + 1));
     }
   }
 };
@@ -158,12 +175,12 @@
   sy_tile_ring<DIAG, SyBuf64<NT>, NP, TP, NBUF>(s, c0, n0, n1, tout, lane);
 }
 
-template <bool NT, int NBUF = 2>
+template <bool NT, int BITS, int NBUF = 2>
 __device__ __forceinline__ void sy_tile_cq(SyLane& s, double scale, double& n0, double& n1, double* __restrict__ tout,
                                            int lane) {
   s.xr0 *= scale;
   s.xr1 *= scale;
-  sy_tile_ring<false, SyBufCq<NT>, true, true, NBUF>(s, 0, n0, n1, tout, lane);
+  sy_tile_ring<false, SyBufCq<NT, BITS>, true, true, NBUF>(s, 0, n0, n1, tout, lane);
   n0 *= scale;
   n1 *= scale;
 }
diff --git a/admm-project_amd/engine.py b/admm-project_amd/engine.py
--- a/admm-project_amd/engine.py
+++ b/admm-project_amd/engine.py
@@ -471,7 +471,8 @@
         ea, eb, diff = C.c_double(), C.c_double(), C.c_double()
         L.check(self._lib.admm_engine_xsolve_storage(self._h, C.byref(form), C.byref(nbytes), C.byref(ea), C.byref(eb),
                                                      C.byref(diff)))
-        return dict(form="compact" if form.value == L.STORAGE_COMPACT else "fp64", stored_bytes=nbytes.value,
+        names = {L.STORAGE_FP64: "fp64", L.STORAGE_COMPACT: "compact", L.STORAGE_COMPACT40: "compact40"}
+        return dict(form=names[form.value], stored_bytes=nbytes.value,
                     probe_err_compact=ea.value, probe_err_fp64=eb.value, probe_diff=diff.value)
 
     def info(self):
diff --git a/include/admm_engine.h b/include/admm_engine.h
--- a/include/admm_engine.h
+++ b/include/admm_engine.h
@@ -240,7 +240,7 @@
   double probe_err_trsv_one;
 } admm_engine_info_t;
 int admm_engine_info(admm_engine* eng, admm_engine_info_t* info);
-enum { ADMM_STORAGE_FP64 = 0, ADMM_STORAGE_COMPACT = 1 };
+enum { ADMM_STORAGE_FP64 = 0, ADMM_STORAGE_COMPACT = 1, ADMM_STORAGE_COMPACT40 = 2 };
 int admm_engine_xsolve_storage(admm_engine* eng, int32_t* form, int64_t* stored_bytes, double* probe_err_compact,
                                double* probe_err_fp64, double* probe_diff);
 int admm_xsolve_compact_accept(double err_compact, double err_fp64, double diff);
@@ -332,6 +332,8 @@
                  int32_t part_count, double* y);
 int admm_op_symv_compact(const double* M, int64_t n, int64_t ldM, const double* x, int32_t fin, int64_t ncached,
                          int32_t part_count, double* y, double* Q, int64_t ldQ);
+int admm_op_symv_compact_bits(const double* M, int64_t n, int64_t ldM, const double* x, int32_t fin, int64_t ncached,
+                              int32_t part_count, double* y, double* Q, int64_t ldQ, int32_t bits);
 int admm_op_symv_batch(const double* Ms, int64_t n, int64_t ldM, int32_t K, const double* X, int64_t ldX,
                        int64_t ncached, double* Y, int64_t ldY);
 int admm_op_gemm(int32_t transA, int32_t transB, int64_t M, int64_t N, int64_t K, double alpha, const double* A,
```

New measurement: 19860 iterations/s, median of 6. 13.6% higher.
